# gnosisguild/stylus-zkvm-verifiers

Measured on NVIDIA B200. Metric: groth16_verifies_per_sec, higher is better.
Workload: dtype u256 (8x32-bit Montgomery limbs, IMAD.WIDE.U32)

## Files before the change

stylus_zkvm_verifiers_b200/csrc/kernels.cuh:

```cuda
#pragma once
#include "bn254.cuh"
#include "lazy.cuh"
#include "sha256.cuh"

namespace zkv {

enum : uint8_t { F_INVALID = 1, F_SKIP0 = 2, F_SKIPC = 4, F_SKIPX = 8, F_SELMIS = 16, F_BADDATA = 32 };
enum : uint8_t { ST_OK = 0, ST_INVALID_INITIALIZATION = 1, ST_INVALID_PROOF_DATA = 2, ST_SELECTOR_MISMATCH = 3, ST_VERIFICATION_FAILED = 4 };

__device__ __forceinline__ uint8_t reject_status(uint8_t fl) { return (fl & F_BADDATA) ? ST_INVALID_PROOF_DATA : (fl & F_SELMIS) ? ST_SELECTOR_MISMATCH : ST_VERIFICATION_FAILED; }
#define F_REJECT (F_INVALID | F_SELMIS | F_BADDATA)

#define ZKV_WIN_BITS 4
#define ZKV_WIN_PER_SCALAR 64
#define ZKV_WIN_ENTRIES 15

struct g1aff { fp x, y; };

__device__ __forceinline__ int g1_decode_raw(fp& x, fp& y, const uint32_t* rx, const uint32_t* ry) {
    if (u256_geq(rx, C_P) || u256_geq(ry, C_P)) return 2;
    uint32_t any = 0;
    for (int i = 0; i < 8; i++) any |= rx[i] | ry[i];
    if (!any) { x = fp_zero(); y = fp_zero(); return 1; }
    fp t;
// ... 54 lines not shown
    const uint8_t* rec = rec_off ? recs + (size_t)(rec_off[i] - rec_base) : recs + (size_t)i * stride;
    const uint64_t len = rec_off ? rec_off[i + 1] - rec_off[i] : (uint64_t)stride;
    uint8_t fl = 0;
    if (rec_off && len < 4) fl = F_BADDATA;
    else if (check_selector) {
        uint32_t s = (uint32_t)rec[0] | (uint32_t)rec[1] << 8 | (uint32_t)rec[2] << 16 | (uint32_t)rec[3] << 24;
        if (s != selector_le) fl = F_SELMIS;
    }
    if (rec_off && !fl && len != off + 256) fl = F_BADDATA;
    if (fl) { decode_reject(i, fl, ax, ay, bx, by, cx, cy, flags); return; }
    decode_points(i, rec + off, vm, ax, ay, bx, by, cx, cy, flags);
}

struct Risc0HashConsts { uint32_t tag_out[8], claim_mid[8], sys0[8]; };
__global__ void k_risc0_signals(int n, const uint8_t* image_ids, const uint8_t* journals, const uint8_t* claims, int mode,
                                Risc0HashConsts hc, uint32_t* scal ) {
    int i = blockIdx.x * blockDim.x + threadIdx.x;
    if (i >= n) return;
    uint32_t claim[8];
    if (mode == 0) {
        uint32_t im[8], jr[8];
        for (int k = 0; k < 8; k++) { im[k] = load_be32(image_ids + 32 * (size_t)i + 4 * k); jr[k] = load_be32(journals + 32 * (size_t)i + 4 * k); }
        risc0_claim_digest(claim, im, jr, hc.tag_out, hc.claim_mid, hc.sys0);
    } else {
        for (int k = 0; k < 8; k++) claim[k] = load_be32(claims + 32 * (size_t)i + 4 * k);
    }
    uint32_t* o = scal + (size_t)i * 16;
    for (int k = 0; k < 4; k++) { o[k] = __byte_perm(claim[k], 0, 0x0123); o[8 + k] = __byte_perm(claim[4 + k], 0, 0x0123); o[4 + k] = 0; o[12 + k] = 0; }
}

__global__ void k_sp1_signals(int n, const uint8_t* vkeys, const uint8_t* pv, const uint64_t* pv_off, uint64_t pv_base, size_t pv_stride,
                              uint32_t* scal , uint8_t* flags) {
    int i = blockIdx.x * blockDim.x + threadIdx.x;
    if (i >= n) return;
    uint32_t* o = scal + (size_t)i * 16;
    uint32_t s0[8];
    be32_to_raw(s0, vkeys + 32 * (size_t)i);
    if (u256_geq(s0, C_R)) flags[i] |= F_INVALID;
    for (int k = 0; k < 8; k++) o[k] = s0[k];
    const uint8_t* msg; size_t len;
    if (pv_off) { msg = pv + (size_t)(pv_off[i] - pv_base); len = (size_t)(pv_off[i + 1] - pv_off[i]); } else { msg = pv + (size_t)i * pv_stride; len = pv_stride; }
    uint32_t h[8];
    sha256_msg(h, msg, len);
    h[0] &= 0x1fffffffu;
    for (int k = 0; k < 8; k++) o[8 + k] = h[7 - k];
}

__global__ void k_generic_signals(int n, int k, const uint8_t* sig, uint32_t* scal, uint8_t* flags) {
    int i = blockIdx.x * blockDim.x + threadIdx.x;
    if (i >= n) return;
    bool bad = false;
    for (int j = 0; j < k; j++) {
        uint32_t s[8];
        be32_to_raw(s, sig + ((size_t)i * k + j) * 32);
        bad |= u256_geq(s, C_R);
        for (int t = 0; t < 8; t++) scal[((size_t)i * k + j) * 8 + t] = s[t];
    }
    if (bad) flags[i] |= F_INVALID;
}

__device__ __forceinline__ void vkx_one(int i, const uint32_t* scal, int stride, int ns, int nwin, const g1aff* tab, const g1aff& base, fp* vx, fp* vy, uint8_t* flags) {
    g1j acc;
    if (fp_is_zero(base.x) && fp_is_zero(base.y)) { acc.x = fp_one(); acc.y = fp_one(); acc.z = fp_zero(); }
    else { acc.x = base.x; acc.y = base.y; acc.z = fp_one(); }
    for (int t = 0; t < ns; t++) {
        const uint32_t* s = scal + ((size_t)i * stride + t) * 8;
        const g1aff* tt = tab + (size_t)t * ZKV_WIN_PER_SCALAR * ZKV_WIN_ENTRIES;
        for (int w = 0; w < nwin; w++) {
            uint32_t d = (s[w >> 3] >> ((w & 7) * 4)) & 15u;
            if (d) {
                const g1aff* e = tt + w * ZKV_WIN_ENTRIES + (d - 1);
                fp ex = e->x, ey = e->y;
                if (!(fp_is_zero(ex) && fp_is_zero(ey))) g1_add_affine(acc, ex, ey);
            }
        }
    }
    fp x, y;
    bool fin = g1_to_affine(x, y, acc);
    vx[i] = x; vy[i] = y;
    if (!fin && flags) flags[i] |= F_SKIPX;
}
__global__ void k_vkx(int n, const uint32_t* scal, int ns, int nwin, const g1aff* tab, g1aff base, fp* vx, fp* vy, uint8_t* flags) {
    int i = blockIdx.x * blockDim.x + threadIdx.x;
    if (i >= n) return;
    vkx_one(i, scal, ns, ns, nwin, tab, base, vx, vy, flags);
}

#if defined(__CUDACC__)
__device__ __noinline__ bool g2v_in_subgroup(fp2 qx, fp2 qy) {
    fp2 X = qx, Y = qy, Z = f2_one();
    const fp2 ny = f2v_neg(qy);
    for (int i = ZKV_U_NAF_LEN - 2; i >= 0; i--) {
        {
            fp2 A = f2v_sqr(X), B = f2v_sqr(Y), C = f2v_sqr(B);
            fp2 D = f2v_dbl(f2v_sub(f2v_sub(f2v_sqr(f2v_add(X, B)), A), C));
            fp2 E = f2v_add(f2v_dbl(A), A), F = f2v_sqr(E);
            fp2 X3 = f2v_sub(F, f2v_dbl(D));
            fp2 Y3 = f2v_sub(f2v_mul(E, f2v_sub(D, X3)), f2v_dbl(f2v_dbl(f2v_dbl(C))));
            Z = f2v_dbl(f2v_mul(Y, Z)); X = X3; Y = Y3;
        }
        const int d = C_U_NAF[i];
        if (d) {
            const fp2 ay = d > 0 ? qy : ny;
            if (f2_is_zero(Z)) { X = qx; Y = ay; Z = f2_one(); continue; }
            fp2 z1z1 = f2v_sqr(Z), u2 = f2v_mul(qx, z1z1), s2 = f2v_mul(f2v_mul(ay, Z), z1z1);
            fp2 h = f2v_sub(u2, X), rr = f2v_sub(s2, Y);
            if (f2_is_zero(h)) {
                if (f2_is_zero(rr)) { g2j p, r; p.x = X; p.y = Y; p.z = Z; g2_dbl(r, p); X = r.x; Y = r.y; Z = r.z; }
                else { X = f2_one(); Y = f2_one(); Z = f2_zero(); }
                continue;
            }
            fp2 hh = f2v_sqr(h), hhh = f2v_mul(hh, h), v = f2v_mul(X, hh);
            fp2 X3 = f2v_sub(f2v_sub(f2v_sqr(rr), hhh), f2v_dbl(v));
            fp2 Y3 = f2v_sub(f2v_mul(rr, f2v_sub(v, X3)), f2v_mul(Y, hhh));
            Z = f2v_mul(Z, h); X = X3; Y = Y3;
        }
    }
    g2j q, uq, lhs, t, p1, p2, p3;
    q.x = qx; q.y = qy; q.z = f2_one(); uq.x = X; uq.y = Y; uq.z = Z;
    g2_add(lhs, uq, q);
    g2_psi(p1, uq, 1); g2_add(t, lhs, p1); lhs = t;
    g2_psi(p2, uq, 2); g2_add(t, lhs, p2); lhs = t;
    g2_dbl(t, uq); g2_psi(p3, t, 3);
    return g2j_eq(lhs, p3);
}
#else
static inline bool g2v_in_subgroup(fp2 qx, fp2 qy) { return g2_in_subgroup(qx, qy); }
#endif
__global__ void k_g2_check(int n, const fp2* bx, const fp2* by, uint8_t* flags) {
    int i = blockIdx.x * blockDim.x + threadIdx.x;
    if (i >= n) return;
    uint8_t fl = flags[i];
    if (fl & F_REJECT) return;
    fp2 x = bx[i], y = by[i];
    if (f2_is_zero(x) && f2_is_zero(y)) return;
    if (!g2v_in_subgroup(x, y)) flags[i] = fl | F_INVALID;
}
__global__ void k_g2_target(int n, const fp2* bx, const fp2* by, fp2* tx, fp2* ty) {
    int i = blockIdx.x * blockDim.x + threadIdx.x;
    if (i >= n) return;
    fp2 x = bx[i], y = by[i];
    g2_neg_psi3(x, y);
    tx[i] = x; ty[i] = y;
}

__global__ void k_or_flags(int n, uint8_t* flags, const uint8_t* extra) {
    int i = blockIdx.x * blockDim.x + threadIdx.x;
    if (i < n && extra[i]) flags[i] |= extra[i];
}

struct MillerArgs {
    const fp* px[4]; const fp* py[4];
    const fp2* qx; const fp2* qy;
    const line_t* tabs[3];
    int nfixed;
    const nline_t* ntabs[2];
    const fp12* pre;
    uint8_t skip_bit[4];
    uint8_t vk_skip;
};
#ifndef ZKV_HTPB
#define ZKV_HTPB 128
#endif
#ifndef ZKV_MINBLOCKS
#define ZKV_MINBLOCKS 2
#endif
#define LZ_SMEM_BYTES (LZ_SLOTS * 32 * LZ_NT)
#define LZ_SMEM_MILLER (LZ_SMEM_BYTES + 1024)
__device__ __noinline__ void lz_slopes_to(fp* sl, const fp* x1, const fp* y1, const fp* x2, const fp* y2, bool off1, bool off2) {
    fp x12[2] = {*x1, *x2}, y12[2] = {*y1, *y2}, xy[2], iy[2];
    bool off[2] = {off1, off2};
    g1_slopes2(xy, iy, x12, y12, off);
    sl[0] = xy[0]; sl[1] = xy[1]; sl[2] = iy[0]; sl[3] = iy[1];
}
__device__ __forceinline__ void miller_lz(int n, const MillerArgs& a, const nline_t* nt0, const nline_t* nt1, const fp12* pre, uint8_t vk_skip,
                                          uint8_t* flags, const fp2* tx, const fp2* ty, fp12* fio, g2j* rst, fp* sl, int d_hi, int d_lo, int first, int last) {
    const int i0 = blockIdx.x * LZ_NT + threadIdx.x, i = i0 < n ? i0 : n - 1;
    const uint8_t fl = flags[i];
    uint32_t skip = vk_skip;
    for (int j = 0; j < 3; j++) if (fl & a.skip_bit[j]) skip |= 1u << j;
    if (fl & F_REJECT) skip = 0xF;
    fp* mysl = sl + 4 * (size_t)i0;
    if (first) lz_slopes_to(mysl, a.px[1] + i, a.py[1] + i, a.px[2] + i, a.py[2] + i, (skip & 2u) != 0, (skip & 4u) != 0);
    LzMillerIn in;
    in.px0 = a.px[0] + i; in.py0 = a.py[0] + i; in.qx = a.qx + i; in.qy = a.qy + i; in.sl = mysl; in.nt[0] = nt0; in.nt[1] = nt1; in.var_off = (skip & 1u) != 0;
    const uint32_t tid = lz_tid();
    if (first) lz_miller_init(a.qx[i], a.qy[i]);
    else {
        lz_ldg12(tid + LZ_F * LZ_SLOT, fio + i);
        const g2j* R = rst + i;
        lz_st2(tid + LZ_R * LZ_SLOT, R->x); lz_st2(tid + (LZ_R + 2) * LZ_SLOT, R->y); lz_st2(tid + (LZ_R + 4) * LZ_SLOT, R->z);
    }
    lz_miller_norm_seg(in, d_hi, d_lo, last != 0);
    if (last && !lz_r_is(tid + LZ_R * LZ_SLOT, tx[i], ty[i]) && i0 < n) flags[i] = fl | F_INVALID;
    if (last) { if (pre) lz_f12mul_g(tid + LZ_F * LZ_SLOT, tid + LZ_T * LZ_SLOT, tid + LZ_R * LZ_SLOT, pre, false); }
    else if (i0 < n) { g2j* R = rst + i; R->x = lz_ld2(tid + LZ_R * LZ_SLOT); R->y = lz_ld2(tid + (LZ_R + 2) * LZ_SLOT); R->z = lz_ld2(tid + (LZ_R + 4) * LZ_SLOT); }
    if (i0 < n) lz_stg12(fio + i, tid + LZ_F * LZ_SLOT);
}
__global__ void __launch_bounds__(LZ_NT, 2) k_miller_lz(int n, MillerArgs a, uint8_t* flags, const fp2* tx, const fp2* ty, fp12* fio, g2j* rst, fp* sl, int d_hi, int d_lo, int first, int last) {
    miller_lz(n, a, a.ntabs[0], a.ntabs[1], a.pre, a.vk_skip, flags, tx, ty, fio, rst, sl, d_hi, d_lo, first, last);
}
__device__ __forceinline__ void final_exp_lz(int n, int s_lo, int s_hi, const fp12* in, fp12* st, const uint8_t* flags, uint8_t* status, uint8_t* gt_out, int pairing_mode) {
    const int i0 = blockIdx.x * LZ_NT + threadIdx.x, i = i0 < n ? i0 : n - 1;
    for (int s = s_lo; s <= s_hi; s++) lz_final_exp_stage(s, in + i, st + 6 * (size_t)i0);
    if (s_hi < 3 || i0 >= n) return;
    const uint8_t fl = flags[i];
    if (fl & (pairing_mode ? (F_INVALID | F_SELMIS) : F_REJECT)) {
        status[i] = pairing_mode ? 2 : reject_status(fl);
        if (gt_out) for (int k = 0; k < 384; k++) gt_out[(size_t)i * 384 + k] = 0;
        return;
    }
    const uint32_t tid = lz_tid();
    fp one = fp_one(); uint32_t t = 0;
    for (int k = 0; k < 12; k++) {
        fp w = lz_ldfp(tid + (LZ_A + k) * LZ_SLOT);
        for (int j = 0; j < 8; j++) t |= w.v[j] ^ (k == 0 ? one.v[j] : 0u);
        if (gt_out) fp_to_be32(gt_out + (size_t)i * 384 + 32 * k, w);
    }
    status[i] = pairing_mode ? (t == 0 ? 1 : 0) : (t == 0 ? ST_OK : ST_VERIFICATION_FAILED);
}
__global__ void __launch_bounds__(LZ_NT, 2) k_final_exp_lz(int n, int s_lo, int s_hi, const fp12* in, fp12* st, const uint8_t* flags, uint8_t* status, uint8_t* gt_out, int pairing_mode) {
    final_exp_lz(n, s_lo, s_hi, in, st, flags, status, gt_out, pairing_mode);
}
__global__ void __launch_bounds__(LZ_NT, 2) k_pairing_lz(int n, LzGenIn in, fp12* fio, int d_hi, int d_lo, int first, int last) {
    const size_t i = (size_t)blockIdx.x * LZ_NT + threadIdx.x;
    const uint32_t tid = lz_tid();
    if (first) { fp2 z = f2_zero(); lz_st2(tid + LZ_F * LZ_SLOT, f2_one()); for (int k = 1; k < 6; k++) lz_st2(tid + (LZ_F + 2 * k) * LZ_SLOT, z); }
    else lz_ldg12(tid + LZ_F * LZ_SLOT, fio + i);
    lz_miller_gen_seg(in, i, d_hi, d_lo, first != 0, last != 0);
    lz_stg12(fio + i, tid + LZ_F * LZ_SLOT);
    (void)n;
}
__global__ void k_pairing4_skip(int n, size_t stride, const uint8_t* flags, uint8_t vk_skip, uint8_t* pskip) {
    int i = blockIdx.x * blockDim.x + threadIdx.x;
    if (i >= n) return;
    const uint8_t fl = flags[i], bits[4] = {F_SKIP0, 0x20, 0x40, 0x80};
    const bool bad = (fl & (F_INVALID | F_SELMIS)) != 0;
    for (int j = 0; j < 4; j++) pskip[(size_t)j * stride + i] = (bad || (fl & bits[j]) || ((vk_skip >> j) & 1)) ? 1 : 0;
}
__global__ void k_pairing_decode(int n, int k, size_t stride, const uint8_t* in, fp* px, fp* py, fp2* qx, fp2* qy, uint8_t* pst) {
    size_t t = (size_t)blockIdx.x * blockDim.x + threadIdx.x;
    if (t >= (size_t)n * k) return;
    const size_t i = t / k; const int j = (int)(t % k);
    const uint8_t* p = in + (i * k + j) * 192;
    uint32_t rx[8], ry[8];
    be32_to_raw(rx, p); be32_to_raw(ry, p + 32);
    fp x, y; int r1 = g1_decode_raw(x, y, rx, ry);
    fp2 x2, y2; int r2 = g2_decode_bytes(x2, y2, p + 64);
    const size_t o = (size_t)j * stride + i;
    px[o] = x; py[o] = y; qx[o] = x2; qy[o] = y2;
    pst[o] = (r1 == 2 || r2 == 2) ? F_INVALID : (r1 == 1 || r2 == 1) ? F_SKIP0 : 0;
}
__global__ void k_pairing_flags(int n, int k, size_t stride, const uint8_t* pst, uint8_t* pskip, uint8_t* iflags) {
    int i = blockIdx.x * blockDim.x + threadIdx.x;
    if (i >= n) return;
    uint8_t bad = 0;
    for (int j = 0; j < k; j++) bad |= pst[(size_t)j * stride + i] & F_INVALID;
    for (int j = 0; j < k; j++) pskip[(size_t)j * stride + i] = (bad || (pst[(size_t)j * stride + i] & F_SKIP0)) ? 1 : 0;
    iflags[i] = bad ? F_INVALID : 0;
}
__global__ void __launch_bounds__(ZKV_HTPB, ZKV_MINBLOCKS) k_fp12_op(int n, int op, const uint8_t* a, const uint8_t* b, uint8_t* out) {
    int i0 = blockIdx.x * blockDim.x + threadIdx.x;
    int i = i0 < n ? i0 : n - 1;
    fp12 x, y, z; fp* xw = &x.c0.c0.c0; fp* yw = &y.c0.c0.c0;
    for (int k = 0; k < 12; k++) {
        fp t; be32_to_raw(t.v, a + (size_t)i * 384 + 32 * k); fp_to_mont(xw[k], t);
        if (b) { be32_to_raw(t.v, b + (size_t)i * 384 + 32 * k); fp_to_mont(yw[k], t); } else yw[k] = fp_zero();
    }
    switch (op) {
        case 0: f12_mul(z, x, y); break;
        case 1: f12_sqr(z, x); break;
        case 2: z = x; f12_mul_line(z, y.c0.c0, y.c0.c1, y.c0.c2); break;
        case 3: f12_cyc_sqr(z, x); break;
        case 4: f12_inv(z, x); break;
        case 5: case 6: case 7: f12_frob(z, x, op - 4); break;
        case 8: final_exp(z, x); break;
        default: {
            fp px[1] = {yw[0]}, py[1] = {yw[1]}; fp2 qx, qy; qx.c1 = yw[2]; qx.c0 = yw[3]; qy.c1 = yw[4]; qy.c0 = yw[5];
            miller_loop(z, px, py, qx, qy, nullptr, 0, n > (1 << 30) ? 1u : 0u); break; }
    }
    if (i0 < n) f12_to_bytes(out + (size_t)i * 384, z);
}
__global__ void __launch_bounds__(LZ_NT, 2) k_lz_fp12_op(int n, int op, const uint8_t* a, const uint8_t* b, uint8_t* out, fp12* scratch , const nline_t* ztab) {
    const int i0 = blockIdx.x * LZ_NT + threadIdx.x, i = i0 < n ? i0 : n - 1;
    const uint32_t tid = lz_tid(), A = tid + LZ_A * LZ_SLOT, X = tid + LZ_X * LZ_SLOT, Y = tid + LZ_Y * LZ_SLOT, L = tid + LZ_L * LZ_SLOT;
    fp12* my = scratch + 7 * (size_t)i0;
    {
        fp12 y; fp* yw = &y.c0.c0.c0;
        for (int k = 0; k < 12; k++) {
            fp t; be32_to_raw(t.v, a + (size_t)i * 384 + 32 * k); fp_to_mont(t, t); lz_stfp(A + k * LZ_SLOT, t);
            if (b) { be32_to_raw(t.v, b + (size_t)i * 384 + 32 * k); fp_to_mont(yw[k], t); } else yw[k] = fp_zero();
        }
        my[6] = y;
    }
    switch (op) {
        case 0: lz_f12mul_g(A, X, Y, my + 6, false); break;
        case 1: lz_f12sqr(A, X); break;
        case 2: { fp2 l0 = my[6].c0.c0; lz_st2(L, my[6].c0.c1); lz_st2(L + 2 * LZ_SLOT, my[6].c0.c2); lz_mul_line(A, X, L, l0); break; }
        case 3: lz_cyc_sqr(A, L); break;
        case 4: lz_f12inv(A, X, Y); break;
        case 5: case 6: case 7: lz_frob(A, op - 4); break;
        case 8: { lz_stg12(my + 6, A); for (int s = 0; s < 4; s++) lz_final_exp_stage(s, my + 6, my); break; }
        case 9: lz_st2(L, my[6].c0.c0); lz_st2(L + 2 * LZ_SLOT, my[6].c0.c1); lz_mul_nline(A, X, L); break;
        default: {
            const fp* yw = &my[6].c0.c0.c0;
            fp* g = &my[0].c0.c0.c0;
            g[0] = yw[0]; g[1] = yw[1]; for (int k = 2; k < 6; k++) g[k] = fp_zero();
            fp2 qx, qy; qx.c1 = yw[2]; qx.c0 = yw[3]; qy.c1 = yw[4]; qy.c0 = yw[5];
            fp2* gq = (fp2*)(g + 6); gq[0] = qx; gq[1] = qy;
            LzMillerIn in; in.px0 = g; in.py0 = g + 1; in.sl = g + 2; in.qx = gq; in.qy = gq + 1; in.nt[0] = ztab; in.nt[1] = ztab; in.var_off = false;
            lz_miller_init(qx, qy);
            const int top = ZKV_ATE_NAF_LEN - 2;
            for (int k = 0; k < 3; k++) lz_miller_norm_seg(in, top - (top + 1) * k / 3, top - (top + 1) * (k + 1) / 3 + 1, k == 2);
            break; }
    }
    if (i0 < n) for (int k = 0; k < 12; k++) fp_to_be32(out + (size_t)i * 384 + 32 * k, lz_ldfp(A + k * LZ_SLOT));
}
__global__ void k_f12_to_bytes(int n, const fp12* in, uint8_t* out) {
    int i = blockIdx.x * blockDim.x + threadIdx.x;
    if (i < n) { fp12 t = in[i]; f12_to_bytes(out + (size_t)i * 384, t); }
}

struct VkDev {
    fp2 g2x[3], g2y[3];
    fp alpha_x, alpha_y;
    int valid;
    int g2_inf[3]; int alpha_inf;
    int norm_ok;
};
__global__ void k_vk_setup(const uint8_t* alpha, const uint8_t* g2bytes , VkDev* vk, line_t* lines , nline_t* nlines ) {
    int j = blockIdx.x;
    if (j < 3) {
        fp2 x, y;
        int r = g2_decode_bytes(x, y, g2bytes + 128 * j);
        if (r == 0 && !g2_in_subgroup(x, y)) r = 2;
        vk->g2x[j] = x; vk->g2y[j] = y; vk->g2_inf[j] = (r == 1);
        if (r == 2) atomicAnd(&vk->valid, 0);
        if (r == 0) g2_precompute_lines(lines + (size_t)j * ZKV_LINES_PER_G2, x, y);
        if (j >= 1 && r == 0 && !g2_normalise_lines(nlines + (size_t)(j - 1) * ZKV_LINES_PER_G2, lines + (size_t)j * ZKV_LINES_PER_G2, ZKV_LINES_PER_G2)) atomicAnd(&vk->norm_ok, 0);
    } else if (j == 3) {
        uint32_t rx[8], ry[8]; be32_to_raw(rx, alpha); be32_to_raw(ry, alpha + 32);
        fp x, y; int r = g1_decode_raw(x, y, rx, ry);
        vk->alpha_x = x; vk->alpha_y = y; vk->alpha_inf = (r == 1);
        if (r == 2) atomicAnd(&vk->valid, 0);
    }
}
__global__ void k_vk_miller_ab(const VkDev* vk, const line_t* lines, fp12* out) {
    fp12 f;
    if (vk->alpha_inf || vk->g2_inf[0] || !vk->valid) { f = f12_one(); }
    else {
        fp px[2], py[2]; px[1] = vk->alpha_x; py[1] = vk->alpha_y; px[0] = fp_zero(); py[0] = fp_zero();
        const line_t* tabs[1] = {lines};
        fp2 z = f2_zero();
        miller_loop(f, px, py, z, z, tabs, 1, 1u);
    }
    *out = f;
}
__global__ void k_ic_tables(const uint8_t* ic , g1aff* tab, g1aff* ic0, VkDev* vk) {
    int t = blockIdx.x, w = threadIdx.x;
    uint32_t rx[8], ry[8];
    if (t == 0 && w == 0) {
        be32_to_raw(rx, ic); be32_to_raw(ry, ic + 32);
        fp x, y; int r = g1_decode_raw(x, y, rx, ry);
        if (r == 2) atomicAnd(&vk->valid, 0);
        ic0->x = x; ic0->y = y;
    }
    be32_to_raw(rx, ic + 64 * (t + 1)); be32_to_raw(ry, ic + 64 * (t + 1) + 32);
    fp x, y; int r = g1_decode_raw(x, y, rx, ry);
    if (r == 2 && w == 0) atomicAnd(&vk->valid, 0);
    g1aff* o = tab + ((size_t)t * ZKV_WIN_PER_SCALAR + w) * ZKV_WIN_ENTRIES;
    if (r != 0) { for (int d = 0; d < ZKV_WIN_ENTRIES; d++) { o[d].x = fp_zero(); o[d].y = fp_zero(); } return; }
    g1j b; b.x = x; b.y = y; b.z = fp_one();
    for (int k = 0; k < ZKV_WIN_BITS * w; k++) { g1j d; g1_dbl(d, b); b = d; }
    fp bx, by; g1_to_affine(bx, by, b);
    g1j acc; acc.x = fp_one(); acc.y = fp_one(); acc.z = fp_zero();
    for (int d = 0; d < ZKV_WIN_ENTRIES; d++) {
        g1_add_affine(acc, bx, by);
        fp ex, ey; g1_to_affine(ex, ey, acc);
        o[d].x = ex; o[d].y = ey;
    }
}

#define ZKV_MAX_KEYS 256
#define ZKV_GROUP_TILE 4096
#define ZKV_SLOT_EMPTY 0xffffffffu
struct KeyDesc {
    g1aff base;
    const g1aff* tab;
    const nline_t* nt[2];
    const fp12* pre;
    int ns, vm, reject;
    uint8_t vk_skip;
};
__device__ __forceinline__ uint32_t group_of(uint32_t k, int nk) { return k < (uint32_t)nk ? k : 0u; }
__global__ void __launch_bounds__(256) k_group_count(int n, int nk, const uint32_t* key_idx, uint32_t* cnt) {
    __shared__ uint32_t h[ZKV_MAX_KEYS];
    for (int k = threadIdx.x; k < nk; k += blockDim.x) h[k] = 0;
    __syncthreads();
    const size_t t0 = (size_t)blockIdx.x * ZKV_GROUP_TILE;
    for (int j = threadIdx.x; j < ZKV_GROUP_TILE; j += blockDim.x)
        if (t0 + j < (size_t)n) atomicAdd(&h[group_of(key_idx[t0 + j], nk)], 1u);
    __syncthreads();
    for (int k = threadIdx.x; k < nk; k += blockDim.x) cnt[(size_t)blockIdx.x * nk + k] = h[k];
}
__global__ void __launch_bounds__(ZKV_MAX_KEYS) k_group_scan(int ntiles, int nk, uint32_t* cnt, uint8_t* slot_key, uint32_t* total) {
    __shared__ uint32_t sc[ZKV_MAX_KEYS];
    const int k = threadIdx.x;
    uint32_t c = 0;
    if (k < nk) for (int t = 0; t < ntiles; t++) c += cnt[(size_t)t * nk + k];
    const uint32_t padded = (c + 31u) & ~31u;
    sc[k] = k < nk ? padded : 0u;
    __syncthreads();
    for (int d = 1; d < ZKV_MAX_KEYS; d <<= 1) {
        const uint32_t v = k >= d ? sc[k - d] : 0u;
        __syncthreads();
        sc[k] += v;
        __syncthreads();
    }
    if (k == ZKV_MAX_KEYS - 1) *total = sc[k];
    if (k >= nk) return;
    uint32_t s = sc[k] - padded;
    for (uint32_t p = s + c; p < s + padded; p++) slot_key[p] = (uint8_t)k;
    for (int t = 0; t < ntiles; t++) { const uint32_t v = cnt[(size_t)t * nk + k]; cnt[(size_t)t * nk + k] = s; s += v; }
}
__global__ void __launch_bounds__(256) k_group_scatter(int n, int nk, const uint32_t* key_idx, const uint32_t* base, uint32_t* perm, uint8_t* slot_key) {
    __shared__ uint32_t wc[8][ZKV_MAX_KEYS];
    const int w = threadIdx.x >> 5, lane = threadIdx.x & 31;
    for (int k = lane; k < nk; k += 32) wc[w][k] = 0;
    __syncwarp();
    const size_t r0 = (size_t)blockIdx.x * ZKV_GROUP_TILE + (size_t)w * (ZKV_GROUP_TILE / 8);
    const unsigned lt = (1u << lane) - 1u;
    for (int r = 0; r < ZKV_GROUP_TILE / 8; r += 32) {
        const size_t i = r0 + r + lane;
        const uint32_t k = i < (size_t)n ? group_of(key_idx[i], nk) : ZKV_SLOT_EMPTY;
        const unsigned peers = __match_any_sync(0xffffffffu, k);
        if (k != ZKV_SLOT_EMPTY && (peers & lt) == 0) wc[w][k] += __popc(peers);
        __syncwarp();
    }
    __syncthreads();
    for (int k = threadIdx.x; k < nk; k += blockDim.x) {
        uint32_t run = base[(size_t)blockIdx.x * nk + k];
        for (int v = 0; v < 8; v++) { const uint32_t c = wc[v][k]; wc[v][k] = run; run += c; }
    }
    __syncthreads();
    for (int r = 0; r < ZKV_GROUP_TILE / 8; r += 32) {
        const size_t i = r0 + r + lane;
        const uint32_t k = i < (size_t)n ? group_of(key_idx[i], nk) : ZKV_SLOT_EMPTY;
        const unsigned peers = __match_any_sync(0xffffffffu, k);
        if (k != ZKV_SLOT_EMPTY) { const uint32_t s = wc[w][k] + __popc(peers & lt); perm[s] = (uint32_t)i; slot_key[s] = (uint8_t)k; }
        __syncwarp();
        if (k != ZKV_SLOT_EMPTY && (peers & lt) == 0) wc[w][k] += __popc(peers);
        __syncwarp();
    }
}
__global__ void k_decode_keys(int n, const uint32_t* perm, const uint8_t* slot_key, const KeyDesc* keys, int nk, const uint32_t* key_idx, const uint8_t* proofs,
                              fp* ax, fp* ay, fp2* bx, fp2* by, fp* cx, fp* cy, uint8_t* flags) {
    int i = blockIdx.x * blockDim.x + threadIdx.x;
    if (i >= n) return;
    const uint32_t p = perm[i];
    const KeyDesc* kd = keys + slot_key[i];
    if (p == ZKV_SLOT_EMPTY || key_idx[p] >= (uint32_t)nk || kd->reject) { decode_reject(i, F_INVALID, ax, ay, bx, by, cx, cy, flags); return; }
    decode_points(i, proofs + (size_t)p * 256, kd->vm, ax, ay, bx, by, cx, cy, flags);
}
__global__ void k_signals_keys(int n, const uint32_t* perm, const uint8_t* slot_key, const KeyDesc* keys, const uint8_t* sig, const uint64_t* sig_off, uint64_t sig_base,
                               int stride, uint32_t* scal, uint8_t* flags) {
    int i = blockIdx.x * blockDim.x + threadIdx.x;
    if (i >= n) return;
    const uint32_t p = perm[i];
    if (p == ZKV_SLOT_EMPTY) return;
    const int k = keys[slot_key[i]].ns;
    const uint64_t a = sig_off[p], b = sig_off[p + 1];
    if (b < a || b - a != (uint64_t)k) { flags[i] |= F_INVALID; return; }
    bool bad = false;
    for (int j = 0; j < k; j++) {
        uint32_t s[8];
        be32_to_raw(s, sig + (a - sig_base + j) * 32);
        bad |= u256_geq(s, C_R);
        for (int t = 0; t < 8; t++) scal[((size_t)i * stride + j) * 8 + t] = s[t];
    }
    if (bad) flags[i] |= F_INVALID;
}
__global__ void k_vkx_keys(int n, const uint32_t* perm, const uint8_t* slot_key, const KeyDesc* keys, const uint32_t* scal, int stride, fp* vx, fp* vy, uint8_t* flags) {
    int i = blockIdx.x * blockDim.x + threadIdx.x;
    if (i >= n) return;
    if (perm[i] == ZKV_SLOT_EMPTY) { vx[i] = fp_zero(); vy[i] = fp_zero(); return; }
    const KeyDesc* kd = keys + slot_key[i];
    const g1aff base = kd->base;
    vkx_one(i, scal, stride, kd->ns, ZKV_WIN_PER_SCALAR, kd->tab, base, vx, vy, flags);
}
__device__ __forceinline__ int grouped_in_chunk(const uint32_t* total, size_t o, int m) {
    const size_t t = *total;
    return t <= o ? 0 : (int)(t - o < (size_t)m ? t - o : (size_t)m);
}
__global__ void __launch_bounds__(LZ_NT, 2) k_miller_lz_keys(const uint32_t* total, size_t o, int m, MillerArgs a, const uint8_t* slot_key, const KeyDesc* keys,
                                                            uint8_t* flags, const fp2* tx, const fp2* ty, fp12* fio, g2j* rst, fp* sl, int d_hi, int d_lo, int first, int last) {
    const int n = grouped_in_chunk(total, o, m);
    if ((int)blockIdx.x * LZ_NT >= n) return;
    const int i0 = blockIdx.x * LZ_NT + threadIdx.x;
    const KeyDesc* kd = keys + slot_key[i0 < n ? i0 : n - 1];
    miller_lz(n, a, kd->nt[0], kd->nt[1], kd->pre, kd->vk_skip, flags, tx, ty, fio, rst, sl, d_hi, d_lo, first, last);
}
__global__ void __launch_bounds__(LZ_NT, 2) k_final_exp_lz_keys(const uint32_t* total, size_t o, int m, int s_lo, int s_hi, const fp12* in, fp12* st, const uint8_t* flags, uint8_t* status) {
    const int n = grouped_in_chunk(total, o, m);
    if ((int)blockIdx.x * LZ_NT >= n) return;
    final_exp_lz(n, s_lo, s_hi, in, st, flags, status, nullptr, 0);
}
__global__ void k_status_to_caller(int n, const uint32_t* total, const uint32_t* perm, const uint8_t* slot_status, uint8_t* status) {
    int i = blockIdx.x * blockDim.x + threadIdx.x;
    if (i >= n || (uint32_t)i >= *total) return;
    const uint32_t p = perm[i];
    if (p != ZKV_SLOT_EMPTY) status[p] = slot_status[i];
}

__global__ void k_g1_decode4(int n, const uint8_t* g1s , const uint8_t* g2s ,
                             fp* px0, fp* py0, fp* px1, fp* py1, fp* px2, fp* py2, fp* px3, fp* py3, fp2* qx, fp2* qy, uint8_t* flags) {
    int i = blockIdx.x * blockDim.x + threadIdx.x;
    if (i >= n) return;
    fp* xs[4] = {px0, px1, px2, px3}; fp* ys[4] = {py0, py1, py2, py3};
    const uint8_t bits[4] = {F_SKIP0, 0x20, 0x40, 0x80};
    uint8_t fl = 0;
    for (int j = 0; j < 4; j++) {
        uint32_t rx[8], ry[8];
        const uint8_t* p = g1s + ((size_t)i * 4 + j) * 64;
        be32_to_raw(rx, p); be32_to_raw(ry, p + 32);
        fp x, y; int r = g1_decode_raw(x, y, rx, ry);
        xs[j][i] = x; ys[j][i] = y;
        if (r == 2) fl |= F_INVALID;
        if (r == 1) fl |= bits[j];
    }
    fp2 x2, y2; int rb = g2_decode_bytes(x2, y2, g2s + (size_t)i * 128);
    qx[i] = x2; qy[i] = y2;
    if (rb == 2) fl |= F_INVALID;
    if (rb == 1) fl |= F_SKIP0;
    flags[i] = fl;
}
__global__ void k_fp_mul_bytes(int n, const uint8_t* a, const uint8_t* b, uint8_t* out) {
    int i = blockIdx.x * blockDim.x + threadIdx.x;
    if (i >= n) return;
    fp x, y, z;
    be32_to_raw(x.v, a + 32 * (size_t)i); be32_to_raw(y.v, b + 32 * (size_t)i);
    fp_to_mont(x, x); fp_to_mont(y, y); fp_mul(z, x, y);
    fp_to_be32(out + 32 * (size_t)i, z);
}
__global__ void k_g2_check_bytes(int n, const uint8_t* g2s, uint8_t* out) {
    int i = blockIdx.x * blockDim.x + threadIdx.x;
    if (i >= n) return;
    fp2 x, y; int r = g2_decode_bytes(x, y, g2s + 128 * (size_t)i);
    if (r == 2) { out[i] = 2; return; }
    if (r == 1) { out[i] = 1; return; }
    out[i] = g2_in_subgroup(x, y) ? 1 : 0;
}
__global__ void k_points_to_bytes(int n, const fp* x, const fp* y, uint8_t* out) {
    int i = blockIdx.x * blockDim.x + threadIdx.x;
    if (i >= n) return;
    fp_to_be32(out + 64 * (size_t)i, x[i]); fp_to_be32(out + 64 * (size_t)i + 32, y[i]);
}


__global__ void k_ec_add(int n, const uint8_t* in, uint8_t* out, uint8_t* ok) {
    int i = blockIdx.x * blockDim.x + threadIdx.x;
    if (i >= n) return;
    const uint8_t* p = in + 128 * (size_t)i;
    uint32_t rx[8], ry[8];
    fp x1, y1, x2, y2;
    be32_to_raw(rx, p); be32_to_raw(ry, p + 32);
    int r1 = g1_decode_raw(x1, y1, rx, ry);
    be32_to_raw(rx, p + 64); be32_to_raw(ry, p + 96);
    int r2 = g1_decode_raw(x2, y2, rx, ry);
    uint8_t* o = out + 64 * (size_t)i;
    if (r1 == 2 || r2 == 2) { ok[i] = 1; for (int k = 0; k < 64; k++) o[k] = 0; return; }
    g1j acc;
    if (r1 == 1) { acc.x = fp_one(); acc.y = fp_one(); acc.z = fp_zero(); } else { acc.x = x1; acc.y = y1; acc.z = fp_one(); }
    if (r2 == 0) g1_add_affine(acc, x2, y2);
    fp x, y; g1_to_affine(x, y, acc);
    fp_to_be32(o, x); fp_to_be32(o + 32, y); ok[i] = 0;
}
__global__ void k_ec_mul(int n, const uint8_t* in, uint8_t* out, uint8_t* ok) {
    int i = blockIdx.x * blockDim.x + threadIdx.x;
    if (i >= n) return;
    const uint8_t* p = in + 96 * (size_t)i;
    uint32_t rx[8], ry[8], s[8];
    fp x1, y1;
    be32_to_raw(rx, p); be32_to_raw(ry, p + 32); be32_to_raw(s, p + 64);
    int r1 = g1_decode_raw(x1, y1, rx, ry);
    uint8_t* o = out + 64 * (size_t)i;
    if (r1 == 2) { ok[i] = 1; for (int k = 0; k < 64; k++) o[k] = 0; return; }
    g1j acc; acc.x = fp_one(); acc.y = fp_one(); acc.z = fp_zero();
    if (r1 == 0) {
        for (int b = 255; b >= 0; b--) {
            g1j d; g1_dbl(d, acc); acc = d;
            if ((s[b >> 5] >> (b & 31)) & 1u) g1_add_affine(acc, x1, y1);
        }
    }
    fp x, y; g1_to_affine(x, y, acc);
    fp_to_be32(o, x); fp_to_be32(o + 32, y); ok[i] = 0;
}
__global__ void k_g2_mul(int n, const uint8_t* pts , int bcast, const uint8_t* scalars, uint8_t* out, uint8_t* ok) {
    int i = blockIdx.x * blockDim.x + threadIdx.x;
    if (i >= n) return;
    fp2 qx, qy; uint32_t s[8];
    int r = g2_decode_bytes(qx, qy, pts + (bcast ? 0 : 128 * (size_t)i));
    be32_to_raw(s, scalars + 32 * (size_t)i);
    uint8_t* o = out + 128 * (size_t)i;
    if (r == 2) { ok[i] = 1; for (int k = 0; k < 128; k++) o[k] = 0; return; }
    g2j acc; acc.x = f2_one(); acc.y = f2_one(); acc.z = f2_zero();
    if (r == 0) {
// ... 39 lines not shown
```

stylus_zkvm_verifiers_b200/csrc/lazy.cuh:

```cuda
#pragma once
#include "bn254.cuh"
#if !defined(__CUDACC__)
#include <cstdio>
#include <cstdlib>
#endif

#ifndef LZ_NT
#define LZ_NT 128
#endif
#define LZ_SLOT (2 * LZ_NT)
#define LZ_SLOTS 28

namespace zkv {

#ifdef LZ_LOCKSTEP
#define LZ_RDV() ZKV_RENDEZVOUS()
#else
#define LZ_RDV()
#endif

struct fp4 { fp2 c0, c1; };

#if defined(__CUDACC__)
#ifndef LZ_FN
#define LZ_FN __device__ __noinline__
#endif
#ifndef LZ_FN2
#define LZ_FN2 __device__ __noinline__
#endif
#define LZ_INL __device__ __forceinline__
extern __shared__ uint4 lz_sm[];
LZ_INL uint32_t lz_tid() { return threadIdx.x; }
#ifdef ZKV_LZ_CHECK
#define LZ_CHK(idx) do { if ((idx) + LZ_NT >= LZ_SLOTS * LZ_SLOT) { printf("smem index out of range: %u (thread %u)\n", (unsigned)(idx), threadIdx.x); return; } } while (0)
#else
#define LZ_CHK(idx)
#endif
LZ_INL void lz_ld(uint32_t* r, uint32_t idx) {
    LZ_CHK(idx);
    uint4 a = lz_sm[idx], b = lz_sm[idx + LZ_NT];
    r[0] = a.x; r[1] = a.y; r[2] = a.z; r[3] = a.w; r[4] = b.x; r[5] = b.y; r[6] = b.z; r[7] = b.w;
}
LZ_INL void lz_st(uint32_t idx, const uint32_t* r) {
    LZ_CHK(idx);
    lz_sm[idx] = make_uint4(r[0], r[1], r[2], r[3]); lz_sm[idx + LZ_NT] = make_uint4(r[4], r[5], r[6], r[7]);
}
#else
#include "../../tests/host_emu/lazy_leaf_host.h"
#endif

LZ_INL void lz_fp_neg(uint32_t* r, const uint32_t* a) { fp z = fp_zero(), x, y; for (int i = 0; i < 8; i++) x.v[i] = a[i]; fp_sub(y, z, x); for (int i = 0; i < 8; i++) r[i] = y.v[i]; }

#include "lazy_gen.cuh"

LZ_INL fp lz_ldfp(uint32_t idx) { fp r; lz_ld(r.v, idx); return r; }
LZ_INL void lz_stfp(uint32_t idx, const fp& a) { lz_st(idx, a.v); }
LZ_INL fp2 lz_ld2(uint32_t idx) { fp2 r; lz_ld(r.c0.v, idx); lz_ld(r.c1.v, idx + LZ_SLOT); return r; }
LZ_INL void lz_st2(uint32_t idx, const fp2& a) { lz_st(idx, a.c0.v); lz_st(idx + LZ_SLOT, a.c1.v); }
LZ_INL void lz_st6(uint32_t idx, const fp6& a) { lz_st2(idx, a.c0); lz_st2(idx + 2 * LZ_SLOT, a.c1); lz_st2(idx + 4 * LZ_SLOT, a.c2); }
LZ_INL fp2 f2v_add(const fp2& a, const fp2& b) { fp2 r; f2_add(r, a, b); return r; }
LZ_INL fp2 f2v_sub(const fp2& a, const fp2& b) { fp2 r; f2_sub(r, a, b); return r; }
LZ_INL fp2 f2v_dbl(const fp2& a) { fp2 r; f2_dbl(r, a); return r; }
LZ_INL fp2 f2v_xi(const fp2& a) {
    fp t0, t1; fp2 r;
    fp_dbl(t0, a.c0); fp_dbl(t0, t0); fp_dbl(t0, t0); fp_add(t0, t0, a.c0);
    fp_dbl(t1, a.c1); fp_dbl(t1, t1); fp_dbl(t1, t1); fp_add(t1, t1, a.c1);
    fp_sub(r.c0, t0, a.c1); fp_add(r.c1, t1, a.c0);
    return r;
}

LZ_FN2 void lz_f12sqr(uint32_t f, uint32_t t) {
    LZ_RDV();
    {
        fp6 ab = lz_f6mul(f, f + 6 * LZ_SLOT);
        lz_st6(t, ab);
    }
    {
        fp2 x0 = lz_ld2(f), x1 = lz_ld2(f + 2 * LZ_SLOT), x2 = lz_ld2(f + 4 * LZ_SLOT);
        fp2 y0 = lz_ld2(f + 6 * LZ_SLOT), y1 = lz_ld2(f + 8 * LZ_SLOT), y2 = lz_ld2(f + 10 * LZ_SLOT);
        lz_st2(f, f2v_add(x0, y0)); lz_st2(f + 2 * LZ_SLOT, f2v_add(x1, y1)); lz_st2(f + 4 * LZ_SLOT, f2v_add(x2, y2));
        lz_st2(f + 6 * LZ_SLOT, f2v_add(x0, f2v_xi(y2))); lz_st2(f + 8 * LZ_SLOT, f2v_add(x1, y0)); lz_st2(f + 10 * LZ_SLOT, f2v_add(x2, y1));
    }
    LZ_RDV();
    fp6 p = lz_f6mul(f, f + 6 * LZ_SLOT);
    fp2 t0 = lz_ld2(t), t1 = lz_ld2(t + 2 * LZ_SLOT), t2 = lz_ld2(t + 4 * LZ_SLOT);
    lz_st2(f, f2v_sub(f2v_sub(p.c0, t0), f2v_xi(t2)));
    lz_st2(f + 2 * LZ_SLOT, f2v_sub(f2v_sub(p.c1, t1), t0));
    lz_st2(f + 4 * LZ_SLOT, f2v_sub(f2v_sub(p.c2, t2), t1));
    lz_st2(f + 6 * LZ_SLOT, f2v_dbl(t0)); lz_st2(f + 8 * LZ_SLOT, f2v_dbl(t1)); lz_st2(f + 10 * LZ_SLOT, f2v_dbl(t2));
}

LZ_FN2 void lz_mul_nline(uint32_t f, uint32_t t, uint32_t l) {
    LZ_RDV();
    { fp6 a = lz_f6mul01(f + 6 * LZ_SLOT, l); lz_st6(t, a); }
    fp6 b = lz_f6mul01(f, l);
    lz_st2(f + 6 * LZ_SLOT, f2v_add(lz_ld2(f + 6 * LZ_SLOT), b.c0));
    lz_st2(f + 8 * LZ_SLOT, f2v_add(lz_ld2(f + 8 * LZ_SLOT), b.c1));
    lz_st2(f + 10 * LZ_SLOT, f2v_add(lz_ld2(f + 10 * LZ_SLOT), b.c2));
    lz_st2(f, f2v_add(lz_ld2(f), f2v_xi(lz_ld2(t + 4 * LZ_SLOT))));
    lz_st2(f + 2 * LZ_SLOT, f2v_add(lz_ld2(f + 2 * LZ_SLOT), lz_ld2(t)));
    lz_st2(f + 4 * LZ_SLOT, f2v_add(lz_ld2(f + 4 * LZ_SLOT), lz_ld2(t + 2 * LZ_SLOT)));
}

LZ_FN fp2 f2v_mul(fp2 a, fp2 b) {
    fp2 r;
#if defined(__CUDA_ARCH__)
    fp2_mul_ptx(r.c0.v, r.c1.v, a.c0.v, a.c1.v, b.c0.v, b.c1.v);
#else
    f2_mul(r, a, b);
#endif
    return r;
}
LZ_FN fp2 f2v_sqr(fp2 a) {
    fp2 r;
#if defined(__CUDA_ARCH__)
    fp2_sqr_ptx(r.c0.v, r.c1.v, a.c0.v, a.c1.v);
#else
    f2_sqr(r, a);
#endif
    return r;
}
LZ_INL fp2 f2v_neg(const fp2& a) { fp2 r; f2_neg(r, a); return r; }
LZ_INL fp2 f2v_half(const fp2& a) { fp2 r; f2_half(r, a); return r; }
LZ_INL fp2 f2v_mul_fp(const fp2& a, const fp& k) { fp2 r; fp_mul(r.c0, a.c0, k); fp_mul(r.c1, a.c1, k); return r; }

LZ_FN2 void lz_mul_line(uint32_t f, uint32_t t, uint32_t l, fp2 a) {
    LZ_RDV();
    { fp6 t1 = lz_f6mul01(f + 6 * LZ_SLOT, l); lz_st6(t, t1); }
    for (int k = 0; k < 3; k++) lz_st2(f + (6 + 2 * k) * LZ_SLOT, f2v_add(lz_ld2(f + 2 * k * LZ_SLOT), lz_ld2(f + (6 + 2 * k) * LZ_SLOT)));
    lz_st2(l, f2v_add(lz_ld2(l), a));
    fp6 s = lz_f6mul01(f + 6 * LZ_SLOT, l);
    {
        fp2 t0 = f2v_mul(lz_ld2(f), a), t10 = lz_ld2(t), t12 = lz_ld2(t + 4 * LZ_SLOT);
        lz_st2(f, f2v_add(t0, f2v_xi(t12)));
        lz_st2(f + 6 * LZ_SLOT, f2v_sub(f2v_sub(s.c0, t0), t10));
        t0 = f2v_mul(lz_ld2(f + 2 * LZ_SLOT), a); fp2 t11 = lz_ld2(t + 2 * LZ_SLOT);
        lz_st2(f + 2 * LZ_SLOT, f2v_add(t0, t10));
        lz_st2(f + 8 * LZ_SLOT, f2v_sub(f2v_sub(s.c1, t0), t11));
        t0 = f2v_mul(lz_ld2(f + 4 * LZ_SLOT), a);
        lz_st2(f + 4 * LZ_SLOT, f2v_add(t0, t11));
        lz_st2(f + 10 * LZ_SLOT, f2v_sub(f2v_sub(s.c2, t0), t12));
    }
}

LZ_INL fp2 lz_line_out(uint32_t l, const fp2& l0, const fp2& l3, const fp2& l4, const fp& px, const fp& py, bool off) {
    fp2 a = f2v_mul_fp(l0, py), b = f2v_mul_fp(l3, px), c = l4;
    const uint32_t keep = off ? 0u : 0xffffffffu;
    for (int k = 0; k < 8; k++) {
        a.c0.v[k] = (a.c0.v[k] & keep) | (C_ONE[k] & ~keep); a.c1.v[k] &= keep;
        b.c0.v[k] &= keep; b.c1.v[k] &= keep; c.c0.v[k] &= keep; c.c1.v[k] &= keep;
    }
    lz_st2(l, b); lz_st2(l + 2 * LZ_SLOT, c);
    return a;
}
LZ_FN2 fp2 lz_line_dbl(uint32_t r, uint32_t l, const fp* px, const fp* py, bool off) {
    LZ_RDV();
    fp2 X = lz_ld2(r), Y = lz_ld2(r + 2 * LZ_SLOT), Z = lz_ld2(r + 4 * LZ_SLOT);
    fp2 A = f2v_half(f2v_mul(X, Y));
    fp2 B = f2v_sqr(Y), C = f2v_sqr(Z);
    fp2 E = f2v_mul(f2_const(C_TWIST_B), f2v_add(f2v_dbl(C), C));
    fp2 F = f2v_add(f2v_dbl(E), E);
    fp2 H = f2v_sub(f2v_sqr(f2v_add(Y, Z)), f2v_add(B, C));
    fp2 J = f2v_sqr(X);
    fp2 E2 = f2v_sqr(E);
    lz_st2(r, f2v_mul(A, f2v_sub(B, F)));
    fp2 G = f2v_sqr(f2v_half(f2v_add(B, F)));
    lz_st2(r + 2 * LZ_SLOT, f2v_sub(G, f2v_add(f2v_dbl(E2), E2)));
    lz_st2(r + 4 * LZ_SLOT, f2v_mul(B, H));
    return lz_line_out(l, f2v_neg(H), f2v_add(f2v_dbl(J), J), f2v_sub(E, B), *px, *py, off);
}
LZ_FN2 fp2 lz_line_add(uint32_t r, uint32_t l, fp2 qx, fp2 qy, const fp* px, const fp* py, bool off) {
    LZ_RDV();
    fp2 X = lz_ld2(r), Y = lz_ld2(r + 2 * LZ_SLOT), Z = lz_ld2(r + 4 * LZ_SLOT);
    fp2 th = f2v_sub(Y, f2v_mul(qy, Z)), la = f2v_sub(X, f2v_mul(qx, Z));
    fp2 C = f2v_sqr(th), D = f2v_sqr(la);
    fp2 E = f2v_mul(la, D), F = f2v_mul(Z, C), G = f2v_mul(X, D);
    fp2 H = f2v_sub(f2v_add(E, F), f2v_dbl(G));
    fp2 l4 = f2v_sub(f2v_mul(th, qx), f2v_mul(la, qy));
    lz_st2(r + 2 * LZ_SLOT, f2v_sub(f2v_mul(th, f2v_sub(G, H)), f2v_mul(E, Y)));
    lz_st2(r, f2v_mul(la, H));
    lz_st2(r + 4 * LZ_SLOT, f2v_mul(Z, E));
    return lz_line_out(l, la, f2v_neg(th), l4, *px, *py, off);
}

#define LZ_F 0
#define LZ_T 12
#define LZ_R 18
#define LZ_L 24
struct LzMillerIn {
    const fp *px0, *py0;
    const fp2 *qx, *qy;
    const fp* sl;
    const nline_t* nt[2];
    bool var_off;
};
#define LZ_STAGE (LZ_SLOTS * LZ_SLOT)
#if defined(__CUDACC__)
LZ_INL uint32_t lz_stage_base() { return LZ_STAGE + (lz_tid() >> 5) * 16; }
LZ_INL uint4 lz_line_fetch(const nline_t* const nt[2], int li) {
    const uint32_t lane = lz_tid() & 31;
    uint4 v = make_uint4(0, 0, 0, 0);
    if (lane < 16) v = ((const uint4*)(nt[lane >> 3] + li))[lane & 7];
    return v;
}
LZ_INL void lz_line_stage(uint4 v) {
    const uint32_t lane = lz_tid() & 31;
    __syncwarp();
    if (lane < 16) lz_sm[lz_stage_base() + lane] = v;
    __syncwarp();
}
LZ_INL nline_t lz_line_staged(int j) {
    nline_t nl; uint4* w = (uint4*)&nl;
    for (int k = 0; k < 8; k++) w[k] = lz_sm[lz_stage_base() + 8 * j + k];
    return nl;
}
#else
struct lz_stage_t { nline_t e[2]; };
static lz_stage_t lz_stage_host;
LZ_INL lz_stage_t lz_line_fetch(const nline_t* const nt[2], int li) { lz_stage_t v; v.e[0] = nt[0][li]; v.e[1] = nt[1][li]; return v; }
LZ_INL void lz_line_stage(const lz_stage_t& v) { lz_stage_host = v; }
LZ_INL nline_t lz_line_staged(int j) { return lz_stage_host.e[j]; }
#endif
LZ_INL void lz_fixed_lines(const LzMillerIn& in, int li, uint32_t tid, bool& have) {
    if (!have) lz_line_stage(lz_line_fetch(in.nt, li));
    const int nx = li + 1 < ZKV_LINES_PER_G2 ? li + 1 : li;
    auto next = lz_line_fetch(in.nt, nx);
    for (int j = 0; j < 2; j++) {
        nline_t nl = lz_line_staged(j);
        lz_st2(tid + LZ_L * LZ_SLOT, f2v_mul_fp(nl.n3, in.sl[j]));
        lz_st2(tid + (LZ_L + 2) * LZ_SLOT, f2v_mul_fp(nl.n4, in.sl[2 + j]));
        lz_mul_nline(tid + LZ_F * LZ_SLOT, tid + LZ_T * LZ_SLOT, tid + LZ_L * LZ_SLOT);
    }
    lz_line_stage(next); have = nx == li + 1;
}
LZ_FN2 void lz_miller_norm_seg(LzMillerIn in, int d_hi, int d_lo, bool last) {
    const uint32_t tid = lz_tid(), F = tid + LZ_F * LZ_SLOT, T = tid + LZ_T * LZ_SLOT, RR = tid + LZ_R * LZ_SLOT, L = tid + LZ_L * LZ_SLOT;
    int li = 0; bool have = false;
    for (int d = ZKV_ATE_NAF_LEN - 2; d > d_hi; d--) li += 1 + (C_ATE_NAF[d] != 0);
    for (int d = d_hi; d >= d_lo; d--) {
        if (d != ZKV_ATE_NAF_LEN - 2) lz_f12sqr(F, T);
        { fp2 a = lz_line_dbl(RR, L, in.px0, in.py0, in.var_off); lz_mul_line(F, T, L, a); }
        lz_fixed_lines(in, li, tid, have);
        li++;
        const int dg = C_ATE_NAF[d];
        if (dg) {
            fp2 y = *in.qy; if (dg < 0) y = f2v_neg(y);
            { fp2 a = lz_line_add(RR, L, *in.qx, y, in.px0, in.py0, in.var_off); lz_mul_line(F, T, L, a); }
            lz_fixed_lines(in, li, tid, have);
            li++;
        }
    }
    if (!last) return;
    for (int s = 1; s <= 2; s++) {
        fp2 xs = *in.qx, ys = *in.qy; g2_frob_affine(xs, ys, s);
        if (s == 2) ys = f2v_neg(ys);
        { fp2 a = lz_line_add(RR, L, xs, ys, in.px0, in.py0, in.var_off); lz_mul_line(F, T, L, a); }
        lz_fixed_lines(in, li, tid, have);
        li++;
    }
}
LZ_INL void g2_neg_psi3(fp2& x, fp2& y) {
    f2_conj(x, x); f2_conj(y, y);
    x = f2v_mul(x, f2_const(C_FROB3[2])); y = f2v_neg(f2v_mul(y, f2_const(C_FROB3[3])));
}
LZ_INL bool lz_r_is(uint32_t r, const fp2& tx, const fp2& ty) {
    const fp2 Z = lz_ld2(r + 4 * LZ_SLOT);
    const fp2 dx = f2v_sub(lz_ld2(r), f2v_mul(tx, Z)), dy = f2v_sub(lz_ld2(r + 2 * LZ_SLOT), f2v_mul(ty, Z));
    return (!f2_is_zero(Z) && f2_is_zero(dx) && f2_is_zero(dy)) || (f2_is_zero(tx) && f2_is_zero(ty));
}
struct LzGenIn {
    const fp *px, *py;
    const fp2 *qx, *qy;
    g2j* rst;
    const line_t* tabs[3];
    const uint8_t* pskip;
    size_t stride; int nvar, nfix;
};
LZ_FN2 void lz_miller_gen_seg(LzGenIn in, size_t i, int d_hi, int d_lo, bool first, bool last) {
    const uint32_t tid = lz_tid(), F = tid + LZ_F * LZ_SLOT, T = tid + LZ_T * LZ_SLOT, RR = tid + LZ_R * LZ_SLOT, L = tid + LZ_L * LZ_SLOT;
    const bool keep = in.nvar == 1;
    int li = 0;
    for (int d = ZKV_ATE_NAF_LEN - 2; d > d_hi; d--) li += 1 + (C_ATE_NAF[d] != 0);
    if (keep) {
        if (first) { lz_st2(RR, in.qx[i]); lz_st2(RR + 2 * LZ_SLOT, in.qy[i]); lz_st2(RR + 4 * LZ_SLOT, f2_one()); }
        else { const g2j* R = in.rst + i; lz_st2(RR, R->x); lz_st2(RR + 2 * LZ_SLOT, R->y); lz_st2(RR + 4 * LZ_SLOT, R->z); }
    }
    const int nsteps = (d_hi - d_lo + 1) + (last ? 2 : 0);
    for (int step = 0; step < nsteps; step++) {
        const int d = d_hi - step;
        const int frob = d < d_lo ? d_lo - d : 0;
        if (!frob && d != ZKV_ATE_NAF_LEN - 2) lz_f12sqr(F, T);
        const int dg = frob ? 1 : C_ATE_NAF[d];
        for (int phase = frob ? 1 : 0; phase < 2; phase++) {
            if (phase == 1 && !dg) break;
            for (int j = 0; j < in.nvar; j++) {
                const size_t ij = (size_t)j * in.stride + i;
                const bool off = in.pskip[ij] != 0;
                if (!keep) {
                    if (first && step == 0 && phase == 0) { lz_st2(RR, in.qx[ij]); lz_st2(RR + 2 * LZ_SLOT, in.qy[ij]); lz_st2(RR + 4 * LZ_SLOT, f2_one()); }
                    else { const g2j* R = in.rst + ij; lz_st2(RR, R->x); lz_st2(RR + 2 * LZ_SLOT, R->y); lz_st2(RR + 4 * LZ_SLOT, R->z); }
                }
                fp2 a;
                if (phase == 0) a = lz_line_dbl(RR, L, in.px + ij, in.py + ij, off);
                else {
                    fp2 x = in.qx[ij], y = in.qy[ij];
                    if (frob) { if (frob == 1) { f2_conj(x, x); f2_conj(y, y); } x = f2v_mul(x, f2_const(frob == 1 ? C_FROB1[2] : C_FROB2[2])); y = f2v_mul(y, f2_const(frob == 1 ? C_FROB1[3] : C_FROB2[3])); if (frob == 2) y = f2v_neg(y); }
                    else if (dg < 0) y = f2v_neg(y);
                    a = lz_line_add(RR, L, x, y, in.px + ij, in.py + ij, off);
                }
                lz_mul_line(F, T, L, a);
                if (!keep) { g2j* R = in.rst + ij; R->x = lz_ld2(RR); R->y = lz_ld2(RR + 2 * LZ_SLOT); R->z = lz_ld2(RR + 4 * LZ_SLOT); }
            }
            for (int j = 0; j < in.nfix; j++) {
                const size_t ij = (size_t)(in.nvar + j) * in.stride + i;
                const line_t ln = in.tabs[j][li];
                fp2 a = lz_line_out(L, ln.l0, ln.l3, ln.l4, in.px[ij], in.py[ij], in.pskip[ij] != 0);
                lz_mul_line(F, T, L, a);
            }
            li++;
        }
    }
    if (keep && !last) { g2j* R = in.rst + i; R->x = lz_ld2(RR); R->y = lz_ld2(RR + 2 * LZ_SLOT); R->z = lz_ld2(RR + 4 * LZ_SLOT); }
}
LZ_INL void lz_miller_init(const fp2& qx, const fp2& qy) {
    const uint32_t tid = lz_tid();
    fp2 one = f2_one(), z = f2_zero();
    lz_st2(tid + LZ_F * LZ_SLOT, one);
    for (int k = 1; k < 6; k++) lz_st2(tid + (LZ_F + 2 * k) * LZ_SLOT, z);
    lz_st2(tid + LZ_R * LZ_SLOT, qx); lz_st2(tid + (LZ_R + 2) * LZ_SLOT, qy); lz_st2(tid + (LZ_R + 4) * LZ_SLOT, one);
}

LZ_INL void lz_ldg6(uint32_t dst, const fp6* src, bool neg) {
    const fp* w = &src->c0.c0;
    for (int k = 0; k < 6; k++) { fp t = w[k]; if (neg) fp_neg(t, t); lz_stfp(dst + k * LZ_SLOT, t); }
}
LZ_INL void lz_ldg12(uint32_t dst, const fp12* src) { lz_ldg6(dst, &src->c0, false); lz_ldg6(dst + 6 * LZ_SLOT, &src->c1, false); }
LZ_INL void lz_stg12(fp12* dst, uint32_t src) { fp* w = &dst->c0.c0.c0; for (int k = 0; k < 12; k++) w[k] = lz_ldfp(src + k * LZ_SLOT); }
LZ_INL void lz_conj(uint32_t a) { for (int k = 6; k < 12; k++) { fp t = lz_ldfp(a + k * LZ_SLOT); fp_neg(t, t); lz_stfp(a + k * LZ_SLOT, t); } }
LZ_FN2 void lz_f12mul_g(uint32_t a, uint32_t x, uint32_t y, const fp12* b, bool conjb) {
    LZ_RDV();
    lz_ldg6(x, &b->c0, false);
    { fp6 t0 = lz_f6mul(a, x); lz_st6(y, t0); }
    for (int k = 0; k < 3; k++) lz_st2(a + 2 * k * LZ_SLOT, f2v_add(lz_ld2(a + 2 * k * LZ_SLOT), lz_ld2(a + (6 + 2 * k) * LZ_SLOT)));
    lz_ldg6(x, &b->c1, conjb);
    { fp6 t1 = lz_f6mul(a + 6 * LZ_SLOT, x); lz_st6(a + 6 * LZ_SLOT, t1); }
    { const fp* w = &b->c0.c0.c0; for (int k = 0; k < 6; k++) { fp t; fp_add(t, lz_ldfp(x + k * LZ_SLOT), w[k]); lz_stfp(x + k * LZ_SLOT, t); } }
    LZ_RDV();
    fp6 m = lz_f6mul(a, x);
    fp2 t10 = lz_ld2(a + 6 * LZ_SLOT), t11 = lz_ld2(a + 8 * LZ_SLOT), t12 = lz_ld2(a + 10 * LZ_SLOT);
    fp2 t00 = lz_ld2(y), t01 = lz_ld2(y + 2 * LZ_SLOT), t02 = lz_ld2(y + 4 * LZ_SLOT);
    lz_st2(a + 6 * LZ_SLOT, f2v_sub(f2v_sub(m.c0, t00), t10));
    lz_st2(a + 8 * LZ_SLOT, f2v_sub(f2v_sub(m.c1, t01), t11));
    lz_st2(a + 10 * LZ_SLOT, f2v_sub(f2v_sub(m.c2, t02), t12));
    lz_st2(a, f2v_add(t00, f2v_xi(t12)));
    lz_st2(a + 2 * LZ_SLOT, f2v_add(t01, t10));
    lz_st2(a + 4 * LZ_SLOT, f2v_add(t02, t11));
}
LZ_FN2 void lz_cyc_sqr(uint32_t a, uint32_t l) {
    LZ_RDV();
    const uint32_t z0 = a, z4 = a + 2 * LZ_SLOT, z3 = a + 4 * LZ_SLOT, z2 = a + 6 * LZ_SLOT, z1 = a + 8 * LZ_SLOT, z5 = a + 10 * LZ_SLOT;
    {
        fp4 t = lz_f4sqr(z0, z1);
        fp2 x = f2v_dbl(f2v_sub(t.c0, lz_ld2(z0))); lz_st2(z0, f2v_add(x, t.c0));
        x = f2v_dbl(f2v_add(t.c1, lz_ld2(z1))); lz_st2(z1, f2v_add(x, t.c1));
    }
    { fp4 t = lz_f4sqr(z2, z3); lz_st2(l, t.c0); lz_st2(l + 2 * LZ_SLOT, t.c1); }
    {
        fp4 t = lz_f4sqr(z4, z5);
        fp2 t5 = f2v_xi(t.c1);
        fp2 x = f2v_dbl(f2v_add(t5, lz_ld2(z2))); lz_st2(z2, f2v_add(x, t5));
        x = f2v_dbl(f2v_sub(t.c0, lz_ld2(z3))); lz_st2(z3, f2v_add(x, t.c0));
        fp2 t2 = lz_ld2(l), t3 = lz_ld2(l + 2 * LZ_SLOT);
        x = f2v_dbl(f2v_sub(t2, lz_ld2(z4))); lz_st2(z4, f2v_add(x, t2));
        x = f2v_dbl(f2v_add(t3, lz_ld2(z5))); lz_st2(z5, f2v_add(x, t3));
    }
}
LZ_FN2 void lz_frob(uint32_t a, int k) {
    LZ_RDV();
    const int slot_of_w[6] = {0, 3, 1, 4, 2, 5};
    for (int i = 0; i < 6; i++) {
        const uint32_t s = a + 2 * slot_of_w[i] * LZ_SLOT;
        fp2 c = lz_ld2(s);
        if (k & 1) f2_conj(c, c);
        if (i) c = f2v_mul(c, (k == 1) ? f2_const(C_FROB1[i]) : (k == 2) ? f2_const(C_FROB2[i]) : f2_const(C_FROB3[i]));
        if (i || (k & 1)) lz_st2(s, c);
    }
}
LZ_INL fp fpv_inv(fp a) { fp r; fp_inv(r, a); return r; }
LZ_FN2 void lz_f12inv(uint32_t a, uint32_t x, uint32_t y) {
    LZ_RDV();
    { fp6 s0 = lz_f6mul(a, a); lz_st6(y, s0); }
    {
        fp6 s1 = lz_f6mul(a + 6 * LZ_SLOT, a + 6 * LZ_SLOT);
        lz_st2(x, f2v_sub(lz_ld2(y), f2v_xi(s1.c2)));
        lz_st2(x + 2 * LZ_SLOT, f2v_sub(lz_ld2(y + 2 * LZ_SLOT), s1.c0));
        lz_st2(x + 4 * LZ_SLOT, f2v_sub(lz_ld2(y + 4 * LZ_SLOT), s1.c1));
    }
    {
        fp2 c0 = lz_ld2(x), c1 = lz_ld2(x + 2 * LZ_SLOT), c2 = lz_ld2(x + 4 * LZ_SLOT);
        fp2 A = f2v_sub(f2v_sqr(c0), f2v_xi(f2v_mul(c1, c2)));
        fp2 B = f2v_sub(f2v_xi(f2v_sqr(c2)), f2v_mul(c0, c1));
        fp2 C = f2v_sub(f2v_sqr(c1), f2v_mul(c0, c2));
        fp2 F = f2v_add(f2v_add(f2v_mul(c0, A), f2v_xi(f2v_mul(c2, B))), f2v_xi(f2v_mul(c1, C)));
        fp n, t; fp_sqr(n, F.c0); fp_sqr(t, F.c1); fp_add(n, n, t); n = fpv_inv(n);
        fp2 Fi; fp_mul(Fi.c0, F.c0, n); fp_mul(t, F.c1, n); fp_neg(Fi.c1, t);
        lz_st2(x, f2v_mul(A, Fi)); lz_st2(x + 2 * LZ_SLOT, f2v_mul(B, Fi)); lz_st2(x + 4 * LZ_SLOT, f2v_mul(C, Fi));
    }
    LZ_RDV();
    { fp6 r0 = lz_f6mul(a, x); lz_st6(a, r0); }
    {
        fp6 r1 = lz_f6mul(a + 6 * LZ_SLOT, x);
        lz_st2(a + 6 * LZ_SLOT, f2v_neg(r1.c0)); lz_st2(a + 8 * LZ_SLOT, f2v_neg(r1.c1)); lz_st2(a + 10 * LZ_SLOT, f2v_neg(r1.c2));
    }
}
#define LZ_A 0
#define LZ_X 12
#define LZ_Y 18
LZ_INL void lz_pow_u(const fp12* ga, fp12* ga3) {
    const uint32_t tid = lz_tid(), A = tid + LZ_A * LZ_SLOT, X = tid + LZ_X * LZ_SLOT, Y = tid + LZ_Y * LZ_SLOT, L = tid + LZ_L * LZ_SLOT;
    lz_ldg12(A, ga);
    lz_cyc_sqr(A, L); lz_f12mul_g(A, X, Y, ga, false);
    lz_stg12(ga3, A);
    if (C_U_WNAF3[ZKV_U_WNAF3_LEN - 1] == 1) lz_ldg12(A, ga);
    for (int i = ZKV_U_WNAF3_LEN - 2; i >= 0; i--) {
        lz_cyc_sqr(A, L);
        const int d = C_U_WNAF3[i];
        if (d) lz_f12mul_g(A, X, Y, (d == 1 || d == -1) ? ga : ga3, d < 0);
    }
}
LZ_INL void lz_final_exp_stage(int stage, const fp12* m, fp12* st) {
    const uint32_t tid = lz_tid(), A = tid + LZ_A * LZ_SLOT, X = tid + LZ_X * LZ_SLOT, Y = tid + LZ_Y * LZ_SLOT, L = tid + LZ_L * LZ_SLOT;
    fp12 *f = st, *s1 = st + 1, *x = st + 2, *y = st + 3, *z = st + 4, *t = st + 5;
    if (stage == 0) {
        lz_ldg12(A, m); lz_f12inv(A, X, Y); lz_f12mul_g(A, X, Y, m, true);
        lz_stg12(f, A); lz_frob(A, 2); lz_f12mul_g(A, X, Y, f, false);
        lz_stg12(f, A);
        lz_pow_u(f, s1);
        lz_stg12(t, A);
    } else if (stage == 1) {
        lz_ldg12(A, t);
        lz_cyc_sqr(A, L); lz_stg12(x, A);
        lz_cyc_sqr(A, L); lz_f12mul_g(A, X, Y, x, false); lz_stg12(y, A);
        lz_pow_u(y, s1); lz_stg12(z, A);
    } else if (stage == 2) {
        lz_ldg12(A, z);
        lz_cyc_sqr(A, L); lz_stg12(t, A);
        lz_pow_u(t, s1);
        lz_stg12(t, A);
    } else {
        lz_ldg12(A, t);
        lz_f12mul_g(A, X, Y, z, false); lz_f12mul_g(A, X, Y, y, false); lz_stg12(t, A);
        lz_f12mul_g(A, X, Y, x, true); lz_stg12(s1, A);
        lz_frob(A, 1); lz_stg12(x, A);
        lz_ldg12(A, s1); lz_f12mul_g(A, X, Y, f, true); lz_frob(A, 3); lz_stg12(s1, A);
        lz_ldg12(A, t); lz_frob(A, 2); lz_stg12(y, A);
        lz_ldg12(A, t); lz_f12mul_g(A, X, Y, z, false); lz_f12mul_g(A, X, Y, f, false);
        lz_f12mul_g(A, X, Y, x, false); lz_f12mul_g(A, X, Y, y, false); lz_f12mul_g(A, X, Y, s1, false);
    }
}

}
```

stylus_zkvm_verifiers_b200/csrc/zkv.cu:

```cuda
#include <cuda_runtime.h>
#include <algorithm>
#include <cstdio>
#include <cstdlib>
#include <cstring>
#include <atomic>
#include <mutex>
#include <string>
#include <thread>
#include <utility>
#include <vector>

#include "../../include/zkv.h"
#include "kernels.cuh"
#include "vk_constants.h"

using namespace zkv;

static thread_local std::string g_err;
static int fail(int code, const std::string& msg) { g_err = msg; return code; }
#define CK(call)                                                                                       \
    do {                                                                                               \
        cudaError_t e_ = (call);                                                                       \
        if (e_ != cudaSuccess) return fail(ZKV_ERR_CUDA, std::string(#call) + ": " + cudaGetErrorString(e_)); \
    } while (0)
// ... 698 lines not shown
        std::lock_guard<std::mutex> lk(c->mu);
        CK(cudaSetDevice(c->device));
        int rc = ctx_wait_idle(c); if (rc) return rc;
        rc = ctx_reserve(c, 1, 24); if (rc) return rc;
        uint32_t sc[24]; memset(sc, 0, sizeof sc);
        uint8_t w32[32];
        memset(w32, 0, 32); memcpy(w32 + 16, h->control_root_0, 16); for (int k = 0; k < 8; k++) sc[k] = load_be32(w32 + 4 * (7 - k));
        memset(w32, 0, 32); memcpy(w32 + 16, h->control_root_1, 16); for (int k = 0; k < 8; k++) sc[8 + k] = load_be32(w32 + 4 * (7 - k));
        for (int k = 0; k < 8; k++) sc[16 + k] = load_be32(bn254_control_id + 4 * (7 - k));
        CK(cudaMemcpyAsync(c->scal, sc, sizeof sc, cudaMemcpyHostToDevice, c->stream));
        CK(cudaMemsetAsync(c->flags, 0, 1, c->stream));
        if (!h->all_fail && h->vk->valid) {
            k_vkx<<<1, 1, 0, c->stream>>>(1, c->scal, 2, ZKV_WIN_PER_SCALAR, c->d_tab, c->h_ic0, c->px[2], c->py[2], c->flags);
            g1aff mid;
            CK(cudaMemcpyAsync(&mid.x, c->px[2], sizeof(fp), cudaMemcpyDeviceToHost, c->stream)); CK(cudaMemcpyAsync(&mid.y, c->py[2], sizeof(fp), cudaMemcpyDeviceToHost, c->stream));
            CK(cudaStreamSynchronize(c->stream));
            k_vkx<<<1, 1, 0, c->stream>>>(1, c->scal + 16, 1, ZKV_WIN_PER_SCALAR, c->d_tab + (size_t)4 * ZKV_WIN_PER_SCALAR * ZKV_WIN_ENTRIES, mid, c->px[2], c->py[2], c->flags);
            CK(cudaMemcpyAsync(&h->base.x, c->px[2], sizeof(fp), cudaMemcpyDeviceToHost, c->stream)); CK(cudaMemcpyAsync(&h->base.y, c->py[2], sizeof(fp), cudaMemcpyDeviceToHost, c->stream));
            CK(cudaStreamSynchronize(c->stream));
            CK(cudaGetLastError());
        } else memset(&h->base, 0, sizeof h->base);
    }
    h->initialized = 1;
    return 0;
}
extern "C" int zkv_risc0_is_initialized(const zkv_risc0* h) { return h ? h->initialized : 0; }
extern "C" int zkv_risc0_get_selector(const zkv_risc0* h, uint8_t out[4]) { if (!h || !out) return fail(ZKV_ERR_ARG, "null"); if (h->initialized) memcpy(out, h->selector, 4); else memset(out, 0, 4); return 0; }
extern "C" int zkv_risc0_get_control_root(const zkv_risc0* h, uint8_t out0[16], uint8_t out1[16]) {
    if (!h || !out0 || !out1) return fail(ZKV_ERR_ARG, "null");
    if (h->initialized) { memcpy(out0, h->control_root_0, 16); memcpy(out1, h->control_root_1, 16); } else { memset(out0, 0, 16); memset(out1, 0, 16); }
    return 0;
}
extern "C" int zkv_risc0_get_bn254_control_id(const zkv_risc0* h, uint8_t out[32]) { if (!h || !out) return fail(ZKV_ERR_ARG, "null"); if (h->initialized) memcpy(out, h->bn254_control_id, 32); else memset(out, 0, 32); return 0; }
extern "C" int zkv_risc0_get_verifier_key_digest(const zkv_risc0* h, uint8_t out[32]) { if (!h || !out) return fail(ZKV_ERR_ARG, "null"); risc0_vk_digest(out, h->vk); return 0; }

static uint32_t sel_le(const uint8_t s[4]) { return (uint32_t)s[0] | (uint32_t)s[1] << 8 | (uint32_t)s[2] << 16 | (uint32_t)s[3] << 24; }
static int risc0_batch(const zkv_risc0* h, const uint8_t* seals, const uint64_t* seal_off, const uint8_t* a32, const uint8_t* b32, int integrity, size_t n, uint8_t* status_out) {
    if (!h || (n && (!seals || !seal_off || !a32 || (!integrity && !b32) || !status_out))) return fail(ZKV_ERR_ARG, "zkv_risc0_verify_batch: null argument");
    if (n == 0) return 0;
    if (n > 0xffffffffull) return fail(ZKV_ERR_ARG, "batch too large");
    if (!offsets_ok(seal_off, n)) return fail(ZKV_ERR_ARG, "seal offsets must be non-decreasing");
    if (!h->initialized) { memset(status_out, ZKV_INVALID_INITIALIZATION, n); return 0; }
    const zkv_vk* vk = h->vk;
    const bool direct = n >= 4096 && is_pinned(seals) && is_pinned(seal_off) && is_pinned(a32) && (integrity || is_pinned(b32));
    const size_t per = integrity ? 32 : 64;
    return for_each_device(vk->devs, n, [&](DevCtx* c, size_t b, size_t e) -> int {
        return host_pipeline(c, vk, b, e, 2, status_out,
            [&](size_t i0, size_t cnt, Sink* dst) -> size_t {
                const size_t bytes = (size_t)(seal_off[i0 + cnt] - seal_off[i0]);
                if (!dst) return (cnt + 1) * 8 + cnt * per + bytes + 320;
                size_t p = 0;
                dst->put(p, seal_off + i0, (cnt + 1) * 8); p += (cnt + 1) * 8;
                dst->put(p, a32 + i0 * 32, cnt * 32); p += cnt * 32;
                if (!integrity) { dst->put(p, b32 + i0 * 32, cnt * 32); p += cnt * 32; }
                dst->put(p, seals + seal_off[i0], bytes, true); p += bytes;
                return p + 320;
            },
            [&](size_t i0, size_t cnt, uint8_t* d) -> Job {
                Job j;
                j.rec_off = (const uint64_t*)d; j.rec_base = seal_off[i0]; j.off = 4; j.stride = 260; j.check_selector = 1; j.selector_le = sel_le(h->selector);
                j.mode = integrity ? SIG_RISC0_INTEGRITY : SIG_RISC0_VERIFY;
                j.sig_a = d + (cnt + 1) * 8; j.sig_b = j.sig_a + cnt * 32; j.recs = j.sig_a + cnt * per;
                j.hc = h->hc; j.base = h->base; j.all_fail = h->all_fail;
                return j;
            }, direct);
    });
}
extern "C" int zkv_risc0_verify_batch(const zkv_risc0* h, const uint8_t* seals, const uint64_t* seal_off, const uint8_t* image_ids, const uint8_t* journal_digests, size_t n, uint8_t* status_out) {
    return risc0_batch(h, seals, seal_off, image_ids, journal_digests, 0, n, status_out);
}
extern "C" int zkv_risc0_verify_integrity_batch(const zkv_risc0* h, const uint8_t* seals, const uint64_t* seal_off, const uint8_t* claim_digests, size_t n, uint8_t* status_out) {
    return risc0_batch(h, seals, seal_off, claim_digests, nullptr, 1, n, status_out);
}
extern "C" int zkv_risc0_verify(const zkv_risc0* h, const uint8_t* seal, size_t seal_len, const uint8_t image_id[32], const uint8_t journal_digest[32], uint8_t* status_out) {
    uint64_t off[2] = {0, seal_len}; uint8_t dummy = 0;
    return risc0_batch(h, seal ? seal : &dummy, off, image_id, journal_digest, 0, 1, status_out);
}
extern "C" int zkv_risc0_verify_integrity(const zkv_risc0* h, const uint8_t* seal, size_t seal_len, const uint8_t claim_digest[32], uint8_t* status_out) {
    uint64_t off[2] = {0, seal_len}; uint8_t dummy = 0;
    return risc0_batch(h, seal ? seal : &dummy, off, claim_digest, nullptr, 1, 1, status_out);
}
extern "C" int zkv_risc0_verify_batch_device(const zkv_risc0* h, int device, const void* d_seals260, const void* d_image_ids, const void* d_journal_digests, size_t n, void* d_status_out, void* stream) {
    if (!h || !d_seals260 || !d_image_ids || !d_journal_digests || !d_status_out) return fail(ZKV_ERR_ARG, "zkv_risc0_verify_batch_device: null argument");
    DevCtx* c = vk_ctx(h->vk, device);
    if (!c) return fail(ZKV_ERR_ARG, "device not in the handle's device list");
    if (n > MAX_CHUNK * 8) return fail(ZKV_ERR_ARG, "device batch too large");
    if (!h->initialized) {
        CK(cudaSetDevice(device));
        CK(cudaMemsetAsync(d_status_out, ZKV_INVALID_INITIALIZATION, n, (cudaStream_t)stream));
        return 0;
    }
    Job j;
    j.vk = h->vk; j.n = n; j.recs = (const uint8_t*)d_seals260; j.stride = 260; j.off = 4; j.check_selector = 1; j.selector_le = sel_le(h->selector);
    j.mode = SIG_RISC0_VERIFY; j.sig_a = (const uint8_t*)d_image_ids; j.sig_b = (const uint8_t*)d_journal_digests; j.hc = h->hc; j.base = h->base; j.all_fail = h->all_fail;
    j.d_status = (uint8_t*)d_status_out;
    return device_call(c, device, stream, [&](cudaStream_t s) { return run_verify(c, j, s); });
}

struct zkv_sp1 { const zkv_vk* vk = nullptr; zkv_vk* owned = nullptr; uint8_t verifier_hash[32]; };
extern "C" int zkv_sp1_create(const zkv_vk* vk_or_null, const int* devices, int n_dev, zkv_sp1** out) {
    if (!out) return fail(ZKV_ERR_ARG, "zkv_sp1_create: null out");
    zkv_sp1* h = new zkv_sp1();
    memcpy(h->verifier_hash, ZKV_SP1_VERIFIER_HASH, 32);
    if (vk_or_null) { if (vk_or_null->n_ic != 3 || vk_or_null->vm != ZKV_VM_SP1) { delete h; return fail(ZKV_ERR_ARG, "zkv_sp1_create: need a ZKV_VM_SP1 key with 3 IC points"); } h->vk = vk_or_null; }
    else { int rc = zkv_vk_load_sp1(devices, n_dev, &h->owned); if (rc) { delete h; return rc; } h->vk = h->owned; }
    *out = h; return 0;
}
extern "C" void zkv_sp1_destroy(zkv_sp1* h) { if (!h) return; if (h->owned) zkv_vk_free(h->owned); delete h; }
extern "C" int zkv_sp1_verifier_hash(const zkv_sp1* h, uint8_t out[32]) { if (!h || !out) return fail(ZKV_ERR_ARG, "null"); memcpy(out, h->verifier_hash, 32); return 0; }
extern "C" const char* zkv_sp1_version(const zkv_sp1*) { return ZKV_SP1_VERSION; }

extern "C" int zkv_sp1_verify_batch(const zkv_sp1* h, const uint8_t* vkeys, const uint8_t* public_values, const uint64_t* pv_off, const uint8_t* proofs, const uint64_t* proof_off, size_t n, uint8_t* status_out) {
    if (!h || (n && (!vkeys || !public_values || !pv_off || !proofs || !proof_off || !status_out))) return fail(ZKV_ERR_ARG, "zkv_sp1_verify_batch: null argument");
    if (n == 0) return 0;
    if (n > 0xffffffffull) return fail(ZKV_ERR_ARG, "batch too large");
    if (!offsets_ok(proof_off, n) || !offsets_ok(pv_off, n)) return fail(ZKV_ERR_ARG, "proof / public-value offsets must be non-decreasing");
    const zkv_vk* vk = h->vk;
    const bool direct = n >= 4096 && is_pinned(proofs) && is_pinned(proof_off) && is_pinned(pv_off) && is_pinned(vkeys) && is_pinned(public_values);
    return for_each_device(vk->devs, n, [&](DevCtx* c, size_t b, size_t e) -> int {
        return host_pipeline(c, vk, b, e, 2, status_out,
            [&](size_t i0, size_t cnt, Sink* dst) -> size_t {
                const size_t pr = (size_t)(proof_off[i0 + cnt] - proof_off[i0]), pv = (size_t)(pv_off[i0 + cnt] - pv_off[i0]);
                if (!dst) return (cnt + 1) * 16 + cnt * 32 + pr + pv + 320;
                size_t p = 0;
                dst->put(p, proof_off + i0, (cnt + 1) * 8); p += (cnt + 1) * 8;
                dst->put(p, pv_off + i0, (cnt + 1) * 8); p += (cnt + 1) * 8;
                dst->put(p, vkeys + i0 * 32, cnt * 32); p += cnt * 32;
                dst->put(p, proofs + proof_off[i0], pr, true); p += pr;
                dst->put(p, public_values + pv_off[i0], pv, true); p += pv;
                return p + 320;
            },
            [&](size_t i0, size_t cnt, uint8_t* d) -> Job {
                Job j;
                j.rec_off = (const uint64_t*)d; j.rec_base = proof_off[i0]; j.off = 4; j.stride = 260; j.check_selector = 1; j.selector_le = sel_le(h->verifier_hash);
                j.mode = SIG_SP1; j.pv_off = (const uint64_t*)(d + (cnt + 1) * 8); j.pv_base = pv_off[i0];
                j.sig_a = d + (cnt + 1) * 16; j.recs = j.sig_a + cnt * 32; j.sig_b = j.recs + (size_t)(proof_off[i0 + cnt] - proof_off[i0]);
                j.base = c->h_ic0;
                return j;
            }, direct);
    });
}
extern "C" int zkv_sp1_verify_proof(const zkv_sp1* h, const uint8_t vkey[32], const uint8_t* public_values, size_t pv_len, const uint8_t* proof, size_t proof_len, uint8_t* status_out) {
    uint64_t po[2] = {0, proof_len}, vo[2] = {0, pv_len}; uint8_t dummy = 0;
    return zkv_sp1_verify_batch(h, vkey, public_values ? public_values : &dummy, vo, proof ? proof : &dummy, po, 1, status_out);
}
extern "C" int zkv_sp1_verify_batch_device(const zkv_sp1* h, int device, const void* d_vkeys, const void* d_public_values, size_t pv_stride, const void* d_proofs260, size_t n, void* d_status_out, void* stream) {
    if (!h || !d_vkeys || !d_public_values || !d_proofs260 || !d_status_out) return fail(ZKV_ERR_ARG, "zkv_sp1_verify_batch_device: null argument");
    DevCtx* c = vk_ctx(h->vk, device);
    if (!c) return fail(ZKV_ERR_ARG, "device not in the handle's device list");
    if (n > MAX_CHUNK * 8) return fail(ZKV_ERR_ARG, "device batch too large");
    Job j;
    j.vk = h->vk; j.n = n; j.recs = (const uint8_t*)d_proofs260; j.stride = 260; j.off = 4; j.check_selector = 1; j.selector_le = sel_le(h->verifier_hash);
    j.mode = SIG_SP1; j.sig_a = (const uint8_t*)d_vkeys; j.sig_b = (const uint8_t*)d_public_values; j.pv_off = nullptr; j.pv_stride = pv_stride; j.base = c->h_ic0;
    j.d_status = (uint8_t*)d_status_out;
    return device_call(c, device, stream, [&](cudaStream_t s) { return run_verify(c, j, s); });
}


extern "C" void zkv_test_parallel_copy(void* dst, const void* src, size_t n) { pcopy(dst, src, n); }
extern "C" void* zkv_host_alloc(size_t bytes) {
    void* p = nullptr;
    if (zkv_device_count() <= 0 || cudaHostAlloc(&p, bytes ? bytes : 1, cudaHostAllocPortable) != cudaSuccess) { cudaGetLastError(); fail(ZKV_ERR_CUDA, "zkv_host_alloc: cudaHostAlloc failed"); return nullptr; }
    return p;
}
extern "C" void zkv_host_free(void* p) { if (p) cudaFreeHost(p); }

extern "C" int zkv_self_test(int device) {
    if (zkv_device_count() <= device || device < 0) return fail(ZKV_ERR_CUDA, "no such CUDA device (this library has no CPU path)");
    zkv_risc0* r0 = nullptr; zkv_sp1* s1 = nullptr;
    int rc = zkv_risc0_create(nullptr, &device, 1, &r0);
    if (!rc) rc = zkv_risc0_initialize(r0, ZKV_RISC0_FIXTURE_CONTROL_ROOT, ZKV_RISC0_FIXTURE_BN254_CONTROL_ID);
    if (!rc) rc = zkv_sp1_create(nullptr, &device, 1, &s1);
    if (!rc) {
        uint8_t st[4] = {255, 255, 255, 255};
        uint8_t seal[sizeof ZKV_RISC0_FIXTURE_SEAL], proof[sizeof ZKV_SP1_FIXTURE_PROOF];
        memcpy(seal, ZKV_RISC0_FIXTURE_SEAL, sizeof seal); memcpy(proof, ZKV_SP1_FIXTURE_PROOF, sizeof proof);
        rc = zkv_risc0_verify(r0, seal, sizeof seal, ZKV_RISC0_FIXTURE_IMAGE_ID, ZKV_RISC0_FIXTURE_JOURNAL_DIGEST, &st[0]);
        seal[4 + 100] ^= 0x04;
        if (!rc) rc = zkv_risc0_verify(r0, seal, sizeof seal, ZKV_RISC0_FIXTURE_IMAGE_ID, ZKV_RISC0_FIXTURE_JOURNAL_DIGEST, &st[1]);
        if (!rc) rc = zkv_sp1_verify_proof(s1, ZKV_SP1_FIXTURE_VKEY, ZKV_SP1_FIXTURE_PUBLIC_VALUES, sizeof ZKV_SP1_FIXTURE_PUBLIC_VALUES, proof, sizeof proof, &st[2]);
        uint8_t vkey[32]; memcpy(vkey, ZKV_SP1_FIXTURE_VKEY, 32); vkey[31] ^= 1;
        if (!rc) rc = zkv_sp1_verify_proof(s1, vkey, ZKV_SP1_FIXTURE_PUBLIC_VALUES, sizeof ZKV_SP1_FIXTURE_PUBLIC_VALUES, proof, sizeof proof, &st[3]);
        if (!rc && !(st[0] == ZKV_OK && st[2] == ZKV_OK && st[1] != ZKV_OK && st[1] != 255 && st[3] == ZKV_VERIFICATION_FAILED)) {
            char msg[160]; snprintf(msg, sizeof msg, "zkv_self_test: kernels returned statuses %d %d %d %d for the reference's golden proofs and their tampers; expected 0, reject, 0, 1", st[0], st[1], st[2], st[3]);
            rc = fail(ZKV_ERR_STATE, msg);
        }
    }
    if (r0) zkv_risc0_destroy(r0);
    if (s1) zkv_sp1_destroy(s1);
    return rc;
}
static int pairing4_chain(DevCtx* c, size_t o, int n, const uint8_t* d_g1s, const uint8_t* d_g2s, uint8_t* d_ok, uint8_t* d_gt, uint8_t* d_miller, cudaStream_t s, bool timed) {
    uint8_t* flags = c->flags + o;
    if (timed) CK(cudaEventRecord(c->ev[0], s));
    k_g1_decode4<<<nblk(n), TPB, 0, s>>>(n, d_g1s + o * 256, d_g2s + o * 128, c->px[0] + o, c->py[0] + o, c->px[1] + o, c->py[1] + o, c->px[2] + o, c->py[2] + o, c->px[3] + o, c->py[3] + o, c->qx + o, c->qy + o, flags);
    if (timed) { CK(cudaEventRecord(c->ev[1], s)); CK(cudaEventRecord(c->ev[2], s)); }
    k_g2_check<<<nblk(n), TPB, 0, s>>>(n, c->qx + o, c->qy + o, flags);
    if (timed) CK(cudaEventRecord(c->ev[3], s));
    const uint8_t vk_skip = (uint8_t)((c->h_vk.g2_inf[0] ? 2 : 0) | (c->h_vk.g2_inf[1] ? 4 : 0) | (c->h_vk.g2_inf[2] ? 8 : 0));
    k_pairing4_skip<<<nblk(n), TPB, 0, s>>>(n, c->stride, flags, vk_skip, c->pskip + o);
    LzGenIn gi; memset(&gi, 0, sizeof gi);
    gi.px = c->px[0] + o; gi.py = c->py[0] + o; gi.qx = c->qx + o; gi.qy = c->qy + o; gi.rst = c->rst + o; gi.pskip = c->pskip + o; gi.stride = c->stride; gi.nvar = 1; gi.nfix = 3;
    for (int j = 0; j < 3; j++) gi.tabs[j] = c->d_lines + (size_t)j * ZKV_LINES_PER_G2;
    k_pairing_lz<<<nblk(n, LZ_NT), LZ_NT, LZ_SMEM_BYTES, s>>>(n, gi, c->f + o, ZKV_ATE_NAF_LEN - 2, 0, 1, 1);
    if (timed) CK(cudaEventRecord(c->ev[4], s));
    if (d_miller) k_f12_to_bytes<<<nblk(n), TPB, 0, s>>>(n, c->f + o, d_miller + o * 384);
    k_final_exp_lz<<<nblk(n, LZ_NT), LZ_NT, LZ_SMEM_BYTES, s>>>(n, 0, 3, c->f + o, c->fes + 6 * o, flags, d_ok + o, d_gt ? d_gt + o * 384 : nullptr, 1);
    if (timed) CK(cudaEventRecord(c->ev[5], s));
    CK(cudaGetLastError());
    return 0;
}
static int run_pairing4(DevCtx* c, const zkv_vk* vk, size_t n_, const uint8_t* d_g1s, const uint8_t* d_g2s, uint8_t* d_ok, uint8_t* d_gt, uint8_t* d_miller, cudaStream_t s) {
    if (n_ == 0) return 0;
    int rc = ctx_acquire(c, s); if (rc) return rc;
    rc = ctx_reserve(c, n_, 8); if (rc) return rc;
    if (!vk->valid) {
        CK(cudaMemsetAsync(d_ok, 2, n_, s)); if (d_gt) CK(cudaMemsetAsync(d_gt, 0, n_ * 384, s)); if (d_miller) CK(cudaMemsetAsync(d_miller, 0, n_ * 384, s));
        for (int e = 0; e < 6; e++) CK(cudaEventRecord(c->ev[e], s));
        return 0;
    }
    int chunks = chunk_count(c, n_, vk->tune.overlap_chunks.load());
    if (vk->tune.overlap_chunks.load() == 0 && n_ >= 2 * wave_proofs_of(c)) chunks = 1;
    if (chunks <= 1) return pairing4_chain(c, 0, (int)n_, d_g1s, d_g2s, d_ok, d_gt, d_miller, s, true);
    return fork_join(c, s, n_, chunks, [&](size_t o, int m, cudaStream_t st) { return pairing4_chain(c, o, m, d_g1s, d_g2s, d_ok, d_gt, d_miller, st, false); });
}
extern "C" int zkv_pairing4_batch(const zkv_vk* vk, const uint8_t* g1s, const uint8_t* g2s, size_t n, uint8_t* ok_out, uint8_t* gt_out, uint8_t* miller_out) {
    if (!vk || (n && (!g1s || !g2s || !ok_out))) return fail(ZKV_ERR_ARG, "zkv_pairing4_batch: null argument");
    if (n == 0) return 0;
    const size_t CH = (size_t)1 << 18;
    return for_each_device(vk->devs, n, [&](DevCtx* c, size_t b, size_t e) -> int {
        if (int rc = ctx_wait_idle(c)) return rc;
        for (size_t s0 = b; s0 < e; s0 += CH) {
            size_t m = std::min(CH, e - s0);
            size_t ob = m + (gt_out ? m * 384 : 0) + (miller_out ? m * 384 : 0);
            int rc = ctx_stage(c, m * 384, ob); if (rc) return rc;
            memcpy(c->h_pin, g1s + s0 * 256, m * 256); memcpy(c->h_pin + m * 256, g2s + s0 * 128, m * 128);
            CK(cudaMemcpyAsync(c->d_in, c->h_pin, m * 384, cudaMemcpyHostToDevice, c->stream));
            uint8_t* d_gt = gt_out ? c->d_out + m : nullptr; uint8_t* d_ml = miller_out ? c->d_out + m + (gt_out ? m * 384 : 0) : nullptr;
            rc = run_pairing4(c, vk, m, c->d_in, c->d_in + m * 256, c->d_out, d_gt, d_ml, c->stream); if (rc) return rc;
            CK(cudaMemcpyAsync(c->h_out, c->d_out, ob, cudaMemcpyDeviceToHost, c->stream));
            CK(cudaStreamSynchronize(c->stream));
            collect_stage_ms(c);
            memcpy(ok_out + s0, c->h_out, m);
            if (gt_out) memcpy(gt_out + s0 * 384, c->h_out + m, m * 384);
            if (miller_out) memcpy(miller_out + s0 * 384, c->h_out + m + (gt_out ? m * 384 : 0), m * 384);
        }
        return 0;
    });
}
extern "C" int zkv_pairing4_batch_device(const zkv_vk* vk, int device, const void* d_g1s, const void* d_g2s, size_t n, void* d_ok_out, void* d_gt_out, void* stream) {
    if (!vk || !d_g1s || !d_g2s || !d_ok_out) return fail(ZKV_ERR_ARG, "zkv_pairing4_batch_device: null argument");
    DevCtx* c = vk_ctx(vk, device);
    if (!c) return fail(ZKV_ERR_ARG, "device not in the key's device list");
    if (n > MAX_CHUNK * 8) return fail(ZKV_ERR_ARG, "device batch too large");
    return device_call(c, device, stream, [&](cudaStream_t s) {
        return run_pairing4(c, vk, n, (const uint8_t*)d_g1s, (const uint8_t*)d_g2s, (uint8_t*)d_ok_out, (uint8_t*)d_gt_out, nullptr, s);
    });
}

extern "C" int zkv_vk_x_batch(const zkv_vk* vk, const uint8_t* signals, int k, size_t n, uint8_t* out_points) {
    if (!vk || !signals || !out_points || k + 1 != vk->n_ic) return fail(ZKV_ERR_ARG, "zkv_vk_x_batch: bad argument");
    if (n == 0) return 0;
    if (n > MAX_CHUNK * 8) return fail(ZKV_ERR_ARG, "zkv_vk_x_batch: batch too large");
    DevCtx* c = vk->devs[0];
    std::lock_guard<std::mutex> lk(c->mu);
    CK(cudaSetDevice(c->device));
    int rc = ctx_wait_idle(c); if (rc) return rc;
    rc = ctx_reserve(c, n, (size_t)k * 8); if (rc) return rc;
    rc = ctx_stage(c, n * (size_t)k * 32, n * 64); if (rc) return rc;
    CK(cudaMemcpyAsync(c->d_in, signals, n * (size_t)k * 32, cudaMemcpyHostToDevice, c->stream));
    CK(cudaMemsetAsync(c->flags, 0, n, c->stream));
    k_generic_signals<<<nblk(n), TPB, 0, c->stream>>>((int)n, k, c->d_in, c->scal, c->flags);
    k_vkx<<<nblk(n), TPB, 0, c->stream>>>((int)n, c->scal, k, ZKV_WIN_PER_SCALAR, c->d_tab, c->h_ic0, c->px[2], c->py[2], c->flags);
    k_points_to_bytes<<<nblk(n), TPB, 0, c->stream>>>((int)n, c->px[2], c->py[2], c->d_out);
    CK(cudaGetLastError());
    CK(cudaMemcpyAsync(out_points, c->d_out, n * 64, cudaMemcpyDeviceToHost, c->stream));
    CK(cudaStreamSynchronize(c->stream));
    return 0;
}

template <class L>
static int with_scratch(int device, const void* in0, size_t b0, const void* in1, size_t b1, void* out0, size_t ob0, void* out1, size_t ob1, L launch) {
    if (zkv_device_count() <= device || device < 0) return fail(ZKV_ERR_CUDA, "no such CUDA device (this library has no CPU path)");
    CK(cudaSetDevice(device));
    uint8_t *d0 = nullptr, *d1 = nullptr, *o0 = nullptr, *o1 = nullptr;
    CK(cudaMalloc(&d0, b0 + 16)); CK(cudaMalloc(&d1, b1 + 16)); CK(cudaMalloc(&o0, ob0 + 16)); CK(cudaMalloc(&o1, ob1 + 16));
    CK(cudaMemcpy(d0, in0, b0, cudaMemcpyHostToDevice)); if (b1) CK(cudaMemcpy(d1, in1, b1, cudaMemcpyHostToDevice));
    launch(d0, d1, o0, o1);
    cudaError_t e = cudaGetLastError(); if (e == cudaSuccess) e = cudaDeviceSynchronize();
    if (e == cudaSuccess) { e = cudaMemcpy(out0, o0, ob0, cudaMemcpyDeviceToHost); if (e == cudaSuccess && ob1) e = cudaMemcpy(out1, o1, ob1, cudaMemcpyDeviceToHost); }
    cudaFree(d0); cudaFree(d1); cudaFree(o0); cudaFree(o1);
    if (e != cudaSuccess) return fail(ZKV_ERR_CUDA, cudaGetErrorString(e));
    return 0;
}
extern "C" int zkv_fp_mul_batch(const uint8_t* a, const uint8_t* b, size_t n, uint8_t* out, int device) {
    if (!a || !b || !out) return fail(ZKV_ERR_ARG, "null");
    if (n == 0) return 0;
    uint8_t dummy;
    return with_scratch(device, a, n * 32, b, n * 32, out, n * 32, &dummy, 0, [&](uint8_t* d0, uint8_t* d1, uint8_t* o0, uint8_t*) { k_fp_mul_bytes<<<nblk(n), TPB>>>((int)n, d0, d1, o0); });
}
extern "C" int zkv_fp12_op_batch(int op, const uint8_t* a, const uint8_t* b, size_t n, uint8_t* out, int device) {
    const bool slots = op >= 16;
    const int k = slots ? op - 16 : op;
    if (!a || !out || k < 0 || k > (slots ? 10 : 9) || ((k == 0 || k == 2 || k == 9 || k == 10) && !b)) return fail(ZKV_ERR_ARG, "zkv_fp12_op_batch: bad argument");
    if (n == 0) return 0;
    uint8_t dummy;
    if (!slots)
        return with_scratch(device, a, n * 384, b ? b : &dummy, b ? n * 384 : 0, out, n * 384, &dummy, 0,
                            [&](uint8_t* d0, uint8_t* d1, uint8_t* o0, uint8_t*) { k_fp12_op<<<nblk(n, ZKV_HTPB), ZKV_HTPB>>>((int)n, k, d0, b ? d1 : nullptr, o0); });
    const size_t launched = (size_t)nblk(n, LZ_NT) * LZ_NT;
    std::vector<uint8_t> sink(1);
    if (zkv_device_count() <= device || device < 0) return fail(ZKV_ERR_CUDA, "no such CUDA device (this library has no CPU path)");
    CK(cudaSetDevice(device));
    CK(cudaFuncSetAttribute(k_lz_fp12_op, cudaFuncAttributeMaxDynamicSharedMemorySize, LZ_SMEM_MILLER));
    fp12* scratch = nullptr; CK(cudaMalloc(&scratch, launched * 7 * sizeof(fp12)));
    nline_t* ztab = nullptr; CK(cudaMalloc(&ztab, ZKV_LINES_PER_G2 * sizeof(nline_t))); CK(cudaMemset(ztab, 0, ZKV_LINES_PER_G2 * sizeof(nline_t)));
    int rc = with_scratch(device, a, n * 384, b ? b : &dummy, b ? n * 384 : 0, out, n * 384, &dummy, 0,
                          [&](uint8_t* d0, uint8_t* d1, uint8_t* o0, uint8_t*) { k_lz_fp12_op<<<nblk(n, LZ_NT), LZ_NT, LZ_SMEM_MILLER>>>((int)n, k, d0, b ? d1 : nullptr, o0, scratch, ztab); });
    cudaFree(scratch); cudaFree(ztab);
    return rc;
}
extern "C" int zkv_g2_check_batch(const uint8_t* g2s, size_t n, uint8_t* out, int device) {
    if (!g2s || !out) return fail(ZKV_ERR_ARG, "null");
    if (n == 0) return 0;
    uint8_t dummy;
    return with_scratch(device, g2s, n * 128, &dummy, 0, out, n, &dummy, 0, [&](uint8_t* d0, uint8_t*, uint8_t* o0, uint8_t*) { k_g2_check_bytes<<<nblk(n), TPB>>>((int)n, d0, o0); });
}
extern "C" int zkv_ec_add_batch(const uint8_t* in, size_t n, uint8_t* out, uint8_t* reverted, int device) {
    if (!in || !out || !reverted) return fail(ZKV_ERR_ARG, "null");
    if (n == 0) return 0;
    uint8_t dummy;
    return with_scratch(device, in, n * 128, &dummy, 0, out, n * 64, reverted, n, [&](uint8_t* d0, uint8_t*, uint8_t* o0, uint8_t* o1) { k_ec_add<<<nblk(n), TPB>>>((int)n, d0, o0, o1); });
}
extern "C" int zkv_ec_mul_batch(const uint8_t* in, size_t n, uint8_t* out, uint8_t* reverted, int device) {
    if (!in || !out || !reverted) return fail(ZKV_ERR_ARG, "null");
    if (n == 0) return 0;
    uint8_t dummy;
    return with_scratch(device, in, n * 96, &dummy, 0, out, n * 64, reverted, n, [&](uint8_t* d0, uint8_t*, uint8_t* o0, uint8_t* o1) { k_ec_mul<<<nblk(n), TPB>>>((int)n, d0, o0, o1); });
}
extern "C" int zkv_g2_mul_batch(const uint8_t* points, int broadcast_point, const uint8_t* scalars, size_t n, uint8_t* out, uint8_t* reverted, int device) {
    if (!points || !scalars || !out || !reverted) return fail(ZKV_ERR_ARG, "null");
    if (n == 0) return 0;
    return with_scratch(device, points, broadcast_point ? 128 : n * 128, scalars, n * 32, out, n * 128, reverted, n,
                        [&](uint8_t* d0, uint8_t* d1, uint8_t* o0, uint8_t* o1) { k_g2_mul<<<nblk(n), TPB>>>((int)n, d0, broadcast_point, d1, o0, o1); });
}
static int ec_pairing_on(int device, const uint8_t* in, int k, size_t n, uint8_t* out, uint8_t* reverted, uint8_t* miller_out) {
    CK(cudaSetDevice(device));
    CK(cudaFuncSetAttribute(k_pairing_lz, cudaFuncAttributeMaxDynamicSharedMemorySize, LZ_SMEM_BYTES));
    CK(cudaFuncSetAttribute(k_final_exp_lz, cudaFuncAttributeMaxDynamicSharedMemorySize, LZ_SMEM_BYTES));
    const size_t CH = (size_t)1 << 16;
    const size_t cap = std::min(CH, (n + LZ_NT - 1) / LZ_NT * LZ_NT), K = (size_t)k;
    uint8_t *d_in = nullptr, *d_pst = nullptr, *d_pskip = nullptr, *d_ifl = nullptr, *d_st = nullptr, *d_ml = nullptr;
    fp *d_px = nullptr, *d_py = nullptr; fp2 *d_qx = nullptr, *d_qy = nullptr; g2j* d_r = nullptr; fp12 *d_f = nullptr, *d_fes = nullptr;
    auto release = [&]() { cudaFree(d_in); cudaFree(d_pst); cudaFree(d_pskip); cudaFree(d_ifl); cudaFree(d_st); cudaFree(d_ml); cudaFree(d_px); cudaFree(d_py); cudaFree(d_qx); cudaFree(d_qy); cudaFree(d_r); cudaFree(d_f); cudaFree(d_fes); };
#define CKR(call) do { cudaError_t e_ = (call); if (e_ != cudaSuccess) { release(); return fail(ZKV_ERR_CUDA, std::string(#call) + ": " + cudaGetErrorString(e_)); } } while (0)
    CKR(cudaMalloc(&d_in, cap * K * 192)); CKR(cudaMalloc(&d_pst, cap * K)); CKR(cudaMalloc(&d_pskip, cap * K)); CKR(cudaMalloc(&d_ifl, cap)); CKR(cudaMalloc(&d_st, cap));
    CKR(cudaMalloc(&d_px, cap * K * sizeof(fp))); CKR(cudaMalloc(&d_py, cap * K * sizeof(fp))); CKR(cudaMalloc(&d_qx, cap * K * sizeof(fp2))); CKR(cudaMalloc(&d_qy, cap * K * sizeof(fp2)));
    CKR(cudaMalloc(&d_r, cap * K * sizeof(g2j))); CKR(cudaMalloc(&d_f, cap * sizeof(fp12))); CKR(cudaMalloc(&d_fes, cap * 6 * sizeof(fp12)));
    if (miller_out) CKR(cudaMalloc(&d_ml, cap * 384));
    std::vector<uint8_t> h_st(cap), h_ifl(cap);
    for (size_t s0 = 0; s0 < n; s0 += CH) {
        const size_t m = std::min(CH, n - s0);
        const int blocks = nblk(m, LZ_NT);
        CKR(cudaMemcpy(d_in, in + s0 * K * 192, m * K * 192, cudaMemcpyHostToDevice));
        CKR(cudaMemset(d_px, 0, cap * K * sizeof(fp))); CKR(cudaMemset(d_py, 0, cap * K * sizeof(fp))); CKR(cudaMemset(d_qx, 0, cap * K * sizeof(fp2))); CKR(cudaMemset(d_qy, 0, cap * K * sizeof(fp2)));
        CKR(cudaMemset(d_pst, F_SKIP0, cap * K)); CKR(cudaMemset(d_pskip, 1, cap * K));
        k_pairing_decode<<<nblk(m * K), TPB>>>((int)m, k, cap, d_in, d_px, d_py, d_qx, d_qy, d_pst);
        k_g2_check<<<nblk(cap * K), TPB>>>((int)(cap * K), d_qx, d_qy, d_pst);
        k_pairing_flags<<<nblk(m), TPB>>>((int)m, k, cap, d_pst, d_pskip, d_ifl);
        LzGenIn gi; memset(&gi, 0, sizeof gi);
        gi.px = d_px; gi.py = d_py; gi.qx = d_qx; gi.qy = d_qy; gi.rst = d_r; gi.pskip = d_pskip; gi.stride = cap; gi.nvar = k; gi.nfix = 0;
        k_pairing_lz<<<blocks, LZ_NT, LZ_SMEM_BYTES>>>((int)m, gi, d_f, ZKV_ATE_NAF_LEN - 2, 0, 1, 1);
        if (miller_out) k_f12_to_bytes<<<nblk(m), TPB>>>((int)m, d_f, d_ml);
        k_final_exp_lz<<<blocks, LZ_NT, LZ_SMEM_BYTES>>>((int)m, 0, 3, d_f, d_fes, d_ifl, d_st, nullptr, 1);
        CKR(cudaGetLastError());
        CKR(cudaMemcpy(h_st.data(), d_st, m, cudaMemcpyDeviceToHost)); CKR(cudaMemcpy(h_ifl.data(), d_ifl, m, cudaMemcpyDeviceToHost));
        if (miller_out) CKR(cudaMemcpy(miller_out + s0 * 384, d_ml, m * 384, cudaMemcpyDeviceToHost));
        for (size_t t = 0; t < m; t++) {
            uint8_t* o = out + (s0 + t) * 32; memset(o, 0, 32);
            if (h_ifl[t]) { reverted[s0 + t] = 1; if (miller_out) memset(miller_out + (s0 + t) * 384, 0, 384); }
            else { reverted[s0 + t] = 0; o[31] = h_st[t] == 1 ? 1 : 0; }
        }
    }
#undef CKR
    release();
    return 0;
}
extern "C" int zkv_ec_pairing_batch(const uint8_t* in, int k, size_t n, uint8_t* out, uint8_t* reverted, uint8_t* miller_out, int device) {
    if (!out || !reverted || k < 0 || k > 64 || (k && n && !in)) return fail(ZKV_ERR_ARG, "zkv_ec_pairing_batch: bad argument");
    if (n == 0) return 0;
    if (zkv_device_count() <= device || device < 0) return fail(ZKV_ERR_CUDA, "no such CUDA device (this library has no CPU path)");
    if (k == 0) {
        for (size_t i = 0; i < n; i++) { memset(out + 32 * i, 0, 32); out[32 * i + 31] = 1; reverted[i] = 0; }
        if (miller_out) for (size_t i = 0; i < n; i++) { memset(miller_out + 384 * i, 0, 384); miller_out[384 * i + 31] = 1; }
        return 0;
    }
    return ec_pairing_on(device, in, k, n, out, reverted, miller_out);
}
extern "C" int zkv_ec_pairing(const uint8_t* in, size_t len, uint8_t out[32], uint8_t* reverted, int device) {
    if (!out || !reverted || (len && !in)) return fail(ZKV_ERR_ARG, "zkv_ec_pairing: null argument");
    if (len % 192) { memset(out, 0, 32); *reverted = 1; return 0; }
    return zkv_ec_pairing_batch(in, (int)(len / 192), 1, out, reverted, nullptr, device);
}

extern "C" int zkv_last_stage_ms(const void* handle_vk, int device, float* out, int cap) {
    const zkv_vk* vk = (const zkv_vk*)handle_vk;
    if (!vk || !out) return fail(ZKV_ERR_ARG, "null");
    DevCtx* c = vk_ctx(vk, device);
    if (!c) return fail(ZKV_ERR_ARG, "device not in the key's device list");
    std::lock_guard<std::mutex> lk(c->mu);
    if (cudaSetDevice(device) == cudaSuccess) { cudaEventSynchronize(c->ev[5]); collect_stage_ms(c); }
    int m = std::min(cap, 5);
    for (int i = 0; i < m; i++) out[i] = c->stage_ms[i];
    return m;
}
extern "C" const void* zkv_risc0_vk(const zkv_risc0* h) { return h ? h->vk : nullptr; }
extern "C" const void* zkv_sp1_vk(const zkv_sp1* h) { return h ? h->vk : nullptr; }

extern "C" long long zkv_wave_proofs(int device, int kernel) {
    if (zkv_device_count() <= device || device < 0) return fail(ZKV_ERR_CUDA, "no such CUDA device");
    if (cudaSetDevice(device) != cudaSuccess) return fail(ZKV_ERR_CUDA, "cudaSetDevice failed");
    cudaDeviceProp prop; if (cudaGetDeviceProperties(&prop, device) != cudaSuccess) return fail(ZKV_ERR_CUDA, "cudaGetDeviceProperties failed");
    int per_sm = 0;
    cudaError_t e; int tpb;
    switch (kernel) {
        case 0: tpb = LZ_NT; cudaFuncSetAttribute(k_miller_lz, cudaFuncAttributeMaxDynamicSharedMemorySize, LZ_SMEM_MILLER); e = cudaOccupancyMaxActiveBlocksPerMultiprocessor(&per_sm, k_miller_lz, LZ_NT, LZ_SMEM_MILLER); break;
        case 1: tpb = LZ_NT; cudaFuncSetAttribute(k_final_exp_lz, cudaFuncAttributeMaxDynamicSharedMemorySize, LZ_SMEM_BYTES); e = cudaOccupancyMaxActiveBlocksPerMultiprocessor(&per_sm, k_final_exp_lz, LZ_NT, LZ_SMEM_BYTES); break;
        default: return fail(ZKV_ERR_ARG, "zkv_wave_proofs: kernel must be 0 or 1 (2 and 3, the round-1 kernels, were removed)");
    }
    if (e != cudaSuccess) return fail(ZKV_ERR_CUDA, cudaGetErrorString(e));
    return (long long)prop.multiProcessorCount * per_sm * tpb;
}
extern "C" int zkv_imad_peak(int device, double* wide_per_s, double* fpmul_per_s) {
    if (zkv_device_count() <= device || device < 0) return fail(ZKV_ERR_CUDA, "no such CUDA device");
    CK(cudaSetDevice(device));
    cudaDeviceProp prop; CK(cudaGetDeviceProperties(&prop, device));
    int blocks = prop.multiProcessorCount * 8, threads = 256;
    uint64_t* d_out; fp* d_fp;
    CK(cudaMalloc(&d_out, (size_t)blocks * threads * 8)); CK(cudaMalloc(&d_fp, (size_t)blocks * threads * sizeof(fp)));
    cudaEvent_t e0, e1; CK(cudaEventCreate(&e0)); CK(cudaEventCreate(&e1));
    float best_w = 1e30f, best_f = 1e30f;
    const int it_w = 4096, it_f = 2048;
    for (int rep = 0; rep < 5; rep++) {
        CK(cudaEventRecord(e0)); k_imad_wide<<<blocks, threads>>>((uint32_t*)d_out, 0x9e3779b9u, 0x7f4a7c15u, it_w); CK(cudaEventRecord(e1)); CK(cudaEventSynchronize(e1));
        float ms; CK(cudaEventElapsedTime(&ms, e0, e1)); if (rep) best_w = std::min(best_w, ms);
        CK(cudaEventRecord(e0)); k_fpmul_chain<<<blocks, threads>>>(d_fp, it_f); CK(cudaEventRecord(e1)); CK(cudaEventSynchronize(e1));
        CK(cudaEventElapsedTime(&ms, e0, e1)); if (rep) best_f = std::min(best_f, ms);
    }
    CK(cudaGetLastError());
    if (wide_per_s) *wide_per_s = (double)blocks * threads * it_w * 64.0 / (best_w * 1e-3);
    if (fpmul_per_s) *fpmul_per_s = (double)blocks * threads * it_f * 2.0 / (best_f * 1e-3);
    cudaEventDestroy(e0); cudaEventDestroy(e1); cudaFree(d_out); cudaFree(d_fp);
    return 0;
}
```

Measured before the change: 2.286 million.

## Generate lazy-reduction G2 line functions and prescale f6 in sparse line multiply

Measured after the change: 2.280 million, median of 6. About the same (-0.3%).

```diff
diff --git a/stylus_zkvm_verifiers_b200/csrc/kernels.cuh b/stylus_zkvm_verifiers_b200/csrc/kernels.cuh
--- a/stylus_zkvm_verifiers_b200/csrc/kernels.cuh
+++ b/stylus_zkvm_verifiers_b200/csrc/kernels.cuh
@@ -380,6 +380,24 @@
         case 5: case 6: case 7: lz_frob(A, op - 4); break;
         case 8: { lz_stg12(my + 6, A); for (int s = 0; s < 4; s++) lz_final_exp_stage(s, my + 6, my); break; }
         case 9: lz_st2(L, my[6].c0.c0); lz_st2(L + 2 * LZ_SLOT, my[6].c0.c1); lz_mul_nline(A, X, L); break;
+        case 16: case 17: {
+            const uint32_t RR = tid + LZ_R * LZ_SLOT;
+            for (int k = 0; k < 6; k++) lz_stfp(RR + k * LZ_SLOT, lz_ldfp(A + k * LZ_SLOT));
+            const bool off = !fp_is_zero(my[6].c0.c0.c0);
+            fp* g = &my[0].c0.c0.c0;
+            fp2 a;
+            if (op == 16) { g[0] = lz_ldfp(A + 6 * LZ_SLOT); g[1] = lz_ldfp(A + 7 * LZ_SLOT); a = lz_line_dbl(RR, L, g, g + 1, off); }
+            else { g[0] = lz_ldfp(A + 10 * LZ_SLOT); g[1] = lz_ldfp(A + 11 * LZ_SLOT); a = lz_line_add(RR, L, lz_ld2(A + 6 * LZ_SLOT), lz_ld2(A + 8 * LZ_SLOT), g, g + 1, off); }
+            for (int k = 0; k < 6; k++) lz_stfp(A + k * LZ_SLOT, lz_ldfp(RR + k * LZ_SLOT));
+            lz_st2(A + 6 * LZ_SLOT, a);
+            for (int k = 0; k < 4; k++) lz_stfp(A + (8 + k) * LZ_SLOT, lz_ldfp(L + k * LZ_SLOT));
+            break; }
+        case 18: lz_f6scale(A, lz_ld2(A + 6 * LZ_SLOT)); break;
+        case 19: {
+            nline_t nl; nl.n3 = lz_ld2(A); nl.n4 = lz_ld2(A + 2 * LZ_SLOT);
+            lz_nline_eval(L, nl, lz_ldfp(A + 4 * LZ_SLOT), lz_ldfp(A + 5 * LZ_SLOT));
+            for (int k = 0; k < 4; k++) lz_stfp(A + k * LZ_SLOT, lz_ldfp(L + k * LZ_SLOT));
+            break; }
         default: {
             const fp* yw = &my[6].c0.c0.c0;
             fp* g = &my[0].c0.c0.c0;
diff --git a/stylus_zkvm_verifiers_b200/csrc/lazy.cuh b/stylus_zkvm_verifiers_b200/csrc/lazy.cuh
--- a/stylus_zkvm_verifiers_b200/csrc/lazy.cuh
+++ b/stylus_zkvm_verifiers_b200/csrc/lazy.cuh
@@ -50,8 +50,10 @@
 #endif
 
 LZ_INL void lz_fp_neg(uint32_t* r, const uint32_t* a) { fp z = fp_zero(), x, y; for (int i = 0; i < 8; i++) x.v[i] = a[i]; fp_sub(y, z, x); for (int i = 0; i < 8; i++) r[i] = y.v[i]; }
+LZ_INL void lz_fp_half(uint32_t* r, const uint32_t* a) { fp x, y; for (int i = 0; i < 8; i++) x.v[i] = a[i]; fp_half(y, x); for (int i = 0; i < 8; i++) r[i] = y.v[i]; }
 
 #include "lazy_gen.cuh"
+#include "lazy_g2_gen.cuh"
 
 LZ_INL fp lz_ldfp(uint32_t idx) { fp r; lz_ld(r.v, idx); return r; }
 LZ_INL void lz_stfp(uint32_t idx, const fp& a) { lz_st(idx, a.v); }
@@ -121,7 +123,6 @@
     return r;
 }
 LZ_INL fp2 f2v_neg(const fp2& a) { fp2 r; f2_neg(r, a); return r; }
-LZ_INL fp2 f2v_half(const fp2& a) { fp2 r; f2_half(r, a); return r; }
 LZ_INL fp2 f2v_mul_fp(const fp2& a, const fp& k) { fp2 r; fp_mul(r.c0, a.c0, k); fp_mul(r.c1, a.c1, k); return r; }
 
 LZ_FN2 void lz_mul_line(uint32_t f, uint32_t t, uint32_t l, fp2 a) {
@@ -129,17 +130,18 @@
     { fp6 t1 = lz_f6mul01(f + 6 * LZ_SLOT, l); lz_st6(t, t1); }
     for (int k = 0; k < 3; k++) lz_st2(f + (6 + 2 * k) * LZ_SLOT, f2v_add(lz_ld2(f + 2 * k * LZ_SLOT), lz_ld2(f + (6 + 2 * k) * LZ_SLOT)));
     lz_st2(l, f2v_add(lz_ld2(l), a));
+    lz_f6scale(f, a);
     fp6 s = lz_f6mul01(f + 6 * LZ_SLOT, l);
     {
-        fp2 t0 = f2v_mul(lz_ld2(f), a), t10 = lz_ld2(t), t12 = lz_ld2(t + 4 * LZ_SLOT);
-        lz_st2(f, f2v_add(t0, f2v_xi(t12)));
-        lz_st2(f + 6 * LZ_SLOT, f2v_sub(f2v_sub(s.c0, t0), t10));
-        t0 = f2v_mul(lz_ld2(f + 2 * LZ_SLOT), a); fp2 t11 = lz_ld2(t + 2 * LZ_SLOT);
-        lz_st2(f + 2 * LZ_SLOT, f2v_add(t0, t10));
-        lz_st2(f + 8 * LZ_SLOT, f2v_sub(f2v_sub(s.c1, t0), t11));
-        t0 = f2v_mul(lz_ld2(f + 4 * LZ_SLOT), a);
-        lz_st2(f + 4 * LZ_SLOT, f2v_add(t0, t11));
-        lz_st2(f + 10 * LZ_SLOT, f2v_sub(f2v_sub(s.c2, t0), t12));
+        fp2 t00 = lz_ld2(f), t10 = lz_ld2(t), t12 = lz_ld2(t + 4 * LZ_SLOT);
+        lz_st2(f, f2v_add(t00, f2v_xi(t12)));
+        lz_st2(f + 6 * LZ_SLOT, f2v_sub(f2v_sub(s.c0, t00), t10));
+        fp2 t01 = lz_ld2(f + 2 * LZ_SLOT), t11 = lz_ld2(t + 2 * LZ_SLOT);
+        lz_st2(f + 2 * LZ_SLOT, f2v_add(t01, t10));
+        lz_st2(f + 8 * LZ_SLOT, f2v_sub(f2v_sub(s.c1, t01), t11));
+        fp2 t02 = lz_ld2(f + 4 * LZ_SLOT);
+        lz_st2(f + 4 * LZ_SLOT, f2v_add(t02, t11));
+        lz_st2(f + 10 * LZ_SLOT, f2v_sub(f2v_sub(s.c2, t02), t12));
     }
 }
 
@@ -152,35 +154,6 @@
     }
     lz_st2(l, b); lz_st2(l + 2 * LZ_SLOT, c);
     return a;
-}
-LZ_FN2 fp2 lz_line_dbl(uint32_t r, uint32_t l, const fp* px, const fp* py, bool off) {
-    LZ_RDV();
-    fp2 X = lz_ld2(r), Y = lz_ld2(r + 2 * LZ_SLOT), Z = lz_ld2(r + 4 * LZ_SLOT);
-    fp2 A = f2v_half(f2v_mul(X, Y));
-    fp2 B = f2v_sqr(Y), C = f2v_sqr(Z);
-    fp2 E = f2v_mul(f2_const(C_TWIST_B), f2v_add(f2v_dbl(C), C));
-    fp2 F = f2v_add(f2v_dbl(E), E);
-    fp2 H = f2v_sub(f2v_sqr(f2v_add(Y, Z)), f2v_add(B, C));
-    fp2 J = f2v_sqr(X);
-    fp2 E2 = f2v_sqr(E);
-    lz_st2(r, f2v_mul(A, f2v_sub(B, F)));
-    fp2 G = f2v_sqr(f2v_half(f2v_add(B, F)));
-    lz_st2(r + 2 * LZ_SLOT, f2v_sub(G, f2v_add(f2v_dbl(E2), E2)));
-    lz_st2(r + 4 * LZ_SLOT, f2v_mul(B, H));
-    return lz_line_out(l, f2v_neg(H), f2v_add(f2v_dbl(J), J), f2v_sub(E, B), *px, *py, off);
-}
-LZ_FN2 fp2 lz_line_add(uint32_t r, uint32_t l, fp2 qx, fp2 qy, const fp* px, const fp* py, bool off) {
-    LZ_RDV();
-    fp2 X = lz_ld2(r), Y = lz_ld2(r + 2 * LZ_SLOT), Z = lz_ld2(r + 4 * LZ_SLOT);
-    fp2 th = f2v_sub(Y, f2v_mul(qy, Z)), la = f2v_sub(X, f2v_mul(qx, Z));
-    fp2 C = f2v_sqr(th), D = f2v_sqr(la);
-    fp2 E = f2v_mul(la, D), F = f2v_mul(Z, C), G = f2v_mul(X, D);
-    fp2 H = f2v_sub(f2v_add(E, F), f2v_dbl(G));
-    fp2 l4 = f2v_sub(f2v_mul(th, qx), f2v_mul(la, qy));
-    lz_st2(r + 2 * LZ_SLOT, f2v_sub(f2v_mul(th, f2v_sub(G, H)), f2v_mul(E, Y)));
-    lz_st2(r, f2v_mul(la, H));
-    lz_st2(r + 4 * LZ_SLOT, f2v_mul(Z, E));
-    return lz_line_out(l, la, f2v_neg(th), l4, *px, *py, off);
 }
 
 #define LZ_F 0
@@ -227,8 +200,7 @@
     auto next = lz_line_fetch(in.nt, nx);
     for (int j = 0; j < 2; j++) {
         nline_t nl = lz_line_staged(j);
-        lz_st2(tid + LZ_L * LZ_SLOT, f2v_mul_fp(nl.n3, in.sl[j]));
-        lz_st2(tid + (LZ_L + 2) * LZ_SLOT, f2v_mul_fp(nl.n4, in.sl[2 + j]));
+        lz_nline_eval(tid + LZ_L * LZ_SLOT, nl, in.sl[j], in.sl[2 + j]);
         lz_mul_nline(tid + LZ_F * LZ_SLOT, tid + LZ_T * LZ_SLOT, tid + LZ_L * LZ_SLOT);
     }
     lz_line_stage(next); have = nx == li + 1;
diff --git a/stylus_zkvm_verifiers_b200/csrc/lazy_g2_gen.cuh b/stylus_zkvm_verifiers_b200/csrc/lazy_g2_gen.cuh
--- /dev/null
+++ b/stylus_zkvm_verifiers_b200/csrc/lazy_g2_gen.cuh
@@ -0,0 +1,471 @@
+#pragma once
+
+LZ_FN fp2 lz_line_dbl(uint32_t r, uint32_t l, const fp* px, const fp* py, bool off) {
+    LZ_RDV();
+    uint32_t n1[8]; lz_ld(n1, r + 0 * LZ_SLOT);
+    uint32_t n2[8]; lz_ld(n2, r + 1 * LZ_SLOT);
+    uint32_t n3[8]; lz_ld(n3, r + 2 * LZ_SLOT);
+    uint32_t n4[8]; lz_ld(n4, r + 3 * LZ_SLOT);
+    uint32_t n5[8]; lz_ld(n5, r + 4 * LZ_SLOT);
+    uint32_t n6[8]; lz_ld(n6, r + 5 * LZ_SLOT);
+    uint32_t n7[8]; lz_add8(n7, n3, n4);
+    uint32_t n8[8]; fp_sub_ptx(n8, n3, n4);
+    uint32_t w9[16]; lz_mulw(w9, n7, n8);
+    uint32_t n10[8]; lz_add8(n10, n3, n3);
+    uint32_t w11[16]; lz_mulw(w11, n10, n4);
+    uint32_t n12[8]; lz_add8(n12, n5, n6);
+    uint32_t n13[8]; fp_sub_ptx(n13, n5, n6);
+    uint32_t w14[16]; lz_mulw(w14, n12, n13);
+    uint32_t n15[8]; lz_add8(n15, n5, n5);
+    uint32_t w16[16]; lz_mulw(w16, n15, n6);
+    uint32_t n17[8]; lz_add8(n17, n1, n2);
+    uint32_t n18[8]; fp_sub_ptx(n18, n1, n2);
+    uint32_t w19[16]; lz_mulw(w19, n17, n18);
+    uint32_t n20[8]; lz_add8(n20, n1, n1);
+    uint32_t w21[16]; lz_mulw(w21, n20, n2);
+    uint32_t n22[8]; lz_add8(n22, n1, n2);
+    uint32_t n23[8]; lz_add8(n23, n3, n4);
+    uint32_t w24[16]; lz_mulw(w24, n22, n23);
+    uint32_t w25[16]; lz_mulw(w25, n1, n3);
+    uint32_t w26[16]; lz_subw(w26, w24, w25);
+    uint32_t w27[16]; lz_mulw(w27, n2, n4);
+    uint32_t w28[16]; lz_subw(w28, w26, w27);
+    uint32_t w29[16]; { const uint32_t c_[9] = {0x950d68e5u, 0xeed1e489u, 0x31469cbeu, 0x61fd4f92u, 0xa6fea8bdu, 0xb4dfc389u, 0xaaf2b553u, 0x7c0f83a2u, 0x0925c4b8u}; lz_addhi(w29, w25, c_); }
+    uint32_t w30[16]; lz_subw(w30, w29, w27);
+    uint32_t n31[8]; lz_redc(n31, w9);
+    { const uint32_t k_[8] = {0xd87cfd47u, 0x3c208c16u, 0x6871ca8du, 0x97816a91u, 0x8181585du, 0xb85045b6u, 0xe131a029u, 0x30644e72u}; lz_csub8(n31, n31, k_); }
+    uint32_t n32[8]; lz_redc(n32, w11);
+    { const uint32_t k_[8] = {0xd87cfd47u, 0x3c208c16u, 0x6871ca8du, 0x97816a91u, 0x8181585du, 0xb85045b6u, 0xe131a029u, 0x30644e72u}; lz_csub8(n32, n32, k_); }
+    uint32_t n33[8]; lz_redc(n33, w14);
+    { const uint32_t k_[8] = {0xd87cfd47u, 0x3c208c16u, 0x6871ca8du, 0x97816a91u, 0x8181585du, 0xb85045b6u, 0xe131a029u, 0x30644e72u}; lz_csub8(n33, n33, k_); }
+    uint32_t n34[8]; lz_redc(n34, w16);
+    { const uint32_t k_[8] = {0xd87cfd47u, 0x3c208c16u, 0x6871ca8du, 0x97816a91u, 0x8181585du, 0xb85045b6u, 0xe131a029u, 0x30644e72u}; lz_csub8(n34, n34, k_); }
+    uint32_t w35[16]; lz_addw(w35, w19, w19);
+    uint32_t w36[16]; lz_addw(w36, w35, w19);
+    uint32_t w37[16]; lz_addw(w37, w21, w21);
+    uint32_t w38[16]; lz_addw(w38, w37, w21);
+    uint32_t n39[8]; lz_redc(n39, w36);
+    { const uint32_t k_[8] = {0xb0f9fa8eu, 0x7841182du, 0xd0e3951au, 0x2f02d522u, 0x0302b0bbu, 0x70a08b6du, 0xc2634053u, 0x60c89ce5u}; lz_csub8(n39, n39, k_); }
+    { const uint32_t k_[8] = {0xd87cfd47u, 0x3c208c16u, 0x6871ca8du, 0x97816a91u, 0x8181585du, 0xb85045b6u, 0xe131a029u, 0x30644e72u}; lz_csub8(n39, n39, k_); }
+    uint32_t n40[8]; lz_redc(n40, w38);
+    { const uint32_t k_[8] = {0xb0f9fa8eu, 0x7841182du, 0xd0e3951au, 0x2f02d522u, 0x0302b0bbu, 0x70a08b6du, 0xc2634053u, 0x60c89ce5u}; lz_csub8(n40, n40, k_); }
+    { const uint32_t k_[8] = {0xd87cfd47u, 0x3c208c16u, 0x6871ca8du, 0x97816a91u, 0x8181585du, 0xb85045b6u, 0xe131a029u, 0x30644e72u}; lz_csub8(n40, n40, k_); }
+    uint32_t n41[8]; lz_redc(n41, w30);
+    { const uint32_t k_[8] = {0xd87cfd47u, 0x3c208c16u, 0x6871ca8du, 0x97816a91u, 0x8181585du, 0xb85045b6u, 0xe131a029u, 0x30644e72u}; lz_csub8(n41, n41, k_); }
+    uint32_t n42[8]; lz_redc(n42, w28);
+    { const uint32_t k_[8] = {0xd87cfd47u, 0x3c208c16u, 0x6871ca8du, 0x97816a91u, 0x8181585du, 0xb85045b6u, 0xe131a029u, 0x30644e72u}; lz_csub8(n42, n42, k_); }
+    uint32_t n43[8]; lz_fp_half(n43, n41);
+    uint32_t n44[8]; lz_fp_half(n44, n42);
+    uint32_t n45[8]; fp_add_ptx(n45, n3, n5);
+    uint32_t n46[8]; fp_add_ptx(n46, n4, n6);
+    uint32_t n47[8]; lz_add8(n47, n45, n46);
+    uint32_t n48[8]; fp_sub_ptx(n48, n45, n46);
+    uint32_t w49[16]; lz_mulw(w49, n47, n48);
+    uint32_t n50[8]; lz_add8(n50, n45, n45);
+    uint32_t w51[16]; lz_mulw(w51, n50, n46);
+    const uint32_t k3b0_[8] = {0xb62e0d6au, 0x3baa927cu, 0xd1b664fdu, 0xd71e7c52u, 0xd95d4664u, 0x03873e63u, 0x082ab8f4u, 0x0e75b5b1u};
+    const uint32_t k3b1_[8] = {0x7596fe35u, 0xaab7c666u, 0xbb6a27bau, 0x31d21a78u, 0x680401ffu, 0x85dd7297u, 0xdf39a7e9u, 0x03c52d6au};
+    uint32_t n52[8]; lz_add8(n52, k3b0_, k3b1_);
+    uint32_t n53[8]; lz_add8(n53, n33, n34);
+    uint32_t w54[16]; lz_mulw(w54, n52, n53);
+    uint32_t w55[16]; lz_mulw(w55, k3b0_, n33);
+    uint32_t w56[16]; lz_subw(w56, w54, w55);
+    uint32_t w57[16]; lz_mulw(w57, k3b1_, n34);
+    uint32_t w58[16]; lz_subw(w58, w56, w57);
+    uint32_t w59[16]; { const uint32_t c_[9] = {0x950d68e5u, 0xeed1e489u, 0x31469cbeu, 0x61fd4f92u, 0xa6fea8bdu, 0xb4dfc389u, 0xaaf2b553u, 0x7c0f83a2u, 0x0925c4b8u}; lz_addhi(w59, w55, c_); }
+    uint32_t w60[16]; lz_subw(w60, w59, w57);
+    uint32_t n61[8]; lz_redc(n61, w60);
+    { const uint32_t k_[8] = {0xd87cfd47u, 0x3c208c16u, 0x6871ca8du, 0x97816a91u, 0x8181585du, 0xb85045b6u, 0xe131a029u, 0x30644e72u}; lz_csub8(n61, n61, k_); }
+    uint32_t n62[8]; lz_redc(n62, w58);
+    { const uint32_t k_[8] = {0xd87cfd47u, 0x3c208c16u, 0x6871ca8du, 0x97816a91u, 0x8181585du, 0xb85045b6u, 0xe131a029u, 0x30644e72u}; lz_csub8(n62, n62, k_); }
+    uint32_t w63[16]; { const uint32_t c_[9] = {0x2a1ad1cau, 0xdda3c913u, 0x628d397du, 0xc3fa9f24u, 0x4dfd517au, 0x69bf8713u, 0x55e56aa7u, 0xf81f0745u, 0x124b8970u}; lz_addhi(w63, w49, c_); }
+    uint32_t w64[16]; lz_subw(w64, w63, w9);
+    uint32_t w65[16]; { const uint32_t c_[9] = {0x2a1ad1cau, 0xdda3c913u, 0x628d397du, 0xc3fa9f24u, 0x4dfd517au, 0x69bf8713u, 0x55e56aa7u, 0xf81f0745u, 0x124b8970u}; lz_addhi(w65, w51, c_); }
+    uint32_t w66[16]; lz_subw(w66, w65, w11);
+    uint32_t w67[16]; { const uint32_t c_[9] = {0x2a1ad1cau, 0xdda3c913u, 0x628d397du, 0xc3fa9f24u, 0x4dfd517au, 0x69bf8713u, 0x55e56aa7u, 0xf81f0745u, 0x124b8970u}; lz_addhi(w67, w64, c_); }
+    uint32_t w68[16]; lz_subw(w68, w67, w14);
+    uint32_t w69[16]; { const uint32_t c_[9] = {0x2a1ad1cau, 0xdda3c913u, 0x628d397du, 0xc3fa9f24u, 0x4dfd517au, 0x69bf8713u, 0x55e56aa7u, 0xf81f0745u, 0x124b8970u}; lz_addhi(w69, w66, c_); }
+    uint32_t w70[16]; lz_subw(w70, w69, w16);
+    uint32_t n71[8]; lz_redc(n71, w68);
+    { const uint32_t k_[8] = {0xb0f9fa8eu, 0x7841182du, 0xd0e3951au, 0x2f02d522u, 0x0302b0bbu, 0x70a08b6du, 0xc2634053u, 0x60c89ce5u}; lz_csub8(n71, n71, k_); }
+    { const uint32_t k_[8] = {0xd87cfd47u, 0x3c208c16u, 0x6871ca8du, 0x97816a91u, 0x8181585du, 0xb85045b6u, 0xe131a029u, 0x30644e72u}; lz_csub8(n71, n71, k_); }
+    uint32_t n72[8]; lz_redc(n72, w70);
+    { const uint32_t k_[8] = {0xb0f9fa8eu, 0x7841182du, 0xd0e3951au, 0x2f02d522u, 0x0302b0bbu, 0x70a08b6du, 0xc2634053u, 0x60c89ce5u}; lz_csub8(n72, n72, k_); }
+    { const uint32_t k_[8] = {0xd87cfd47u, 0x3c208c16u, 0x6871ca8du, 0x97816a91u, 0x8181585du, 0xb85045b6u, 0xe131a029u, 0x30644e72u}; lz_csub8(n72, n72, k_); }
+    uint32_t n73[8]; fp_add_ptx(n73, n61, n61);
+    uint32_t n74[8]; fp_add_ptx(n74, n62, n62);
+    uint32_t n75[8]; fp_add_ptx(n75, n73, n61);
+    uint32_t n76[8]; fp_add_ptx(n76, n74, n62);
+    uint32_t n77[8]; fp_add_ptx(n77, n31, n75);
+    uint32_t n78[8]; fp_add_ptx(n78, n32, n76);
+    uint32_t n79[8]; lz_fp_half(n79, n77);
+    uint32_t n80[8]; lz_fp_half(n80, n78);
+    uint32_t n81[8]; lz_add8(n81, n61, n62);
+    uint32_t n82[8]; fp_sub_ptx(n82, n61, n62);
+    uint32_t w83[16]; lz_mulw(w83, n81, n82);
+    uint32_t n84[8]; lz_add8(n84, n61, n61);
+    uint32_t w85[16]; lz_mulw(w85, n84, n62);
+    uint32_t n86[8]; lz_add8(n86, n79, n80);
+    uint32_t n87[8]; fp_sub_ptx(n87, n79, n80);
+    uint32_t w88[16]; lz_mulw(w88, n86, n87);
+    uint32_t n89[8]; lz_add8(n89, n79, n79);
+    uint32_t w90[16]; lz_mulw(w90, n89, n80);
+    uint32_t w91[16]; lz_addw(w91, w83, w83);
+    uint32_t w92[16]; lz_addw(w92, w91, w83);
+    uint32_t w93[16]; lz_addw(w93, w85, w85);
+    uint32_t w94[16]; lz_addw(w94, w93, w85);
+    uint32_t w95[16]; { const uint32_t c_[9] = {0x7e50755eu, 0x98eb5b39u, 0x27a7ac79u, 0x4befdd6du, 0xe9f7f470u, 0x3d3e9539u, 0x01b03ff6u, 0xe85d15d0u, 0x36e29c52u}; lz_addhi(w95, w88, c_); }
+    uint32_t w96[16]; lz_subw(w96, w95, w92);
+    uint32_t w97[16]; { const uint32_t c_[9] = {0x7e50755eu, 0x98eb5b39u, 0x27a7ac79u, 0x4befdd6du, 0xe9f7f470u, 0x3d3e9539u, 0x01b03ff6u, 0xe85d15d0u, 0x36e29c52u}; lz_addhi(w97, w90, c_); }
+    uint32_t w98[16]; lz_subw(w98, w97, w94);
+    uint32_t n99[8]; lz_redc(n99, w96);
+    { const uint32_t k_[8] = {0xb0f9fa8eu, 0x7841182du, 0xd0e3951au, 0x2f02d522u, 0x0302b0bbu, 0x70a08b6du, 0xc2634053u, 0x60c89ce5u}; lz_csub8(n99, n99, k_); }
+    { const uint32_t k_[8] = {0xd87cfd47u, 0x3c208c16u, 0x6871ca8du, 0x97816a91u, 0x8181585du, 0xb85045b6u, 0xe131a029u, 0x30644e72u}; lz_csub8(n99, n99, k_); }
+    uint32_t n100[8]; lz_redc(n100, w98);
+    { const uint32_t k_[8] = {0xb0f9fa8eu, 0x7841182du, 0xd0e3951au, 0x2f02d522u, 0x0302b0bbu, 0x70a08b6du, 0xc2634053u, 0x60c89ce5u}; lz_csub8(n100, n100, k_); }
+    { const uint32_t k_[8] = {0xd87cfd47u, 0x3c208c16u, 0x6871ca8du, 0x97816a91u, 0x8181585du, 0xb85045b6u, 0xe131a029u, 0x30644e72u}; lz_csub8(n100, n100, k_); }
+    uint32_t n101[8]; fp_sub_ptx(n101, n31, n75);
+    uint32_t n102[8]; fp_sub_ptx(n102, n32, n76);
+    uint32_t n103[8]; lz_add8(n103, n43, n44);
+    uint32_t n104[8]; lz_add8(n104, n101, n102);
+    uint32_t w105[16]; lz_mulw(w105, n103, n104);
+    uint32_t w106[16]; lz_mulw(w106, n43, n101);
+    uint32_t w107[16]; lz_subw(w107, w105, w106);
+    uint32_t w108[16]; lz_mulw(w108, n44, n102);
+    uint32_t w109[16]; lz_subw(w109, w107, w108);
+    uint32_t w110[16]; { const uint32_t c_[9] = {0x950d68e5u, 0xeed1e489u, 0x31469cbeu, 0x61fd4f92u, 0xa6fea8bdu, 0xb4dfc389u, 0xaaf2b553u, 0x7c0f83a2u, 0x0925c4b8u}; lz_addhi(w110, w106, c_); }
+    uint32_t w111[16]; lz_subw(w111, w110, w108);
+    uint32_t n112[8]; lz_redc(n112, w111);
+    { const uint32_t k_[8] = {0xd87cfd47u, 0x3c208c16u, 0x6871ca8du, 0x97816a91u, 0x8181585du, 0xb85045b6u, 0xe131a029u, 0x30644e72u}; lz_csub8(n112, n112, k_); }
+    uint32_t n113[8]; lz_redc(n113, w109);
+    { const uint32_t k_[8] = {0xd87cfd47u, 0x3c208c16u, 0x6871ca8du, 0x97816a91u, 0x8181585du, 0xb85045b6u, 0xe131a029u, 0x30644e72u}; lz_csub8(n113, n113, k_); }
+    uint32_t n114[8]; lz_add8(n114, n31, n32);
+    uint32_t n115[8]; lz_add8(n115, n71, n72);
+    uint32_t w116[16]; lz_mulw(w116, n114, n115);
+    uint32_t w117[16]; lz_mulw(w117, n31, n71);
+    uint32_t w118[16]; lz_subw(w118, w116, w117);
+    uint32_t w119[16]; lz_mulw(w119, n32, n72);
+    uint32_t w120[16]; lz_subw(w120, w118, w119);
+    uint32_t w121[16]; { const uint32_t c_[9] = {0x950d68e5u, 0xeed1e489u, 0x31469cbeu, 0x61fd4f92u, 0xa6fea8bdu, 0xb4dfc389u, 0xaaf2b553u, 0x7c0f83a2u, 0x0925c4b8u}; lz_addhi(w121, w117, c_); }
+    uint32_t w122[16]; lz_subw(w122, w121, w119);
+    uint32_t n123[8]; lz_redc(n123, w122);
+    { const uint32_t k_[8] = {0xd87cfd47u, 0x3c208c16u, 0x6871ca8du, 0x97816a91u, 0x8181585du, 0xb85045b6u, 0xe131a029u, 0x30644e72u}; lz_csub8(n123, n123, k_); }
+    uint32_t n124[8]; lz_redc(n124, w120);
+    { const uint32_t k_[8] = {0xd87cfd47u, 0x3c208c16u, 0x6871ca8du, 0x97816a91u, 0x8181585du, 0xb85045b6u, 0xe131a029u, 0x30644e72u}; lz_csub8(n124, n124, k_); }
+    uint32_t n125[8]; lz_fp_neg(n125, n71);
+    uint32_t n126[8]; lz_fp_neg(n126, n72);
+    uint32_t w127[16]; lz_mulw(w127, n125, py->v);
+    uint32_t n128[8]; lz_redc(n128, w127);
+    { const uint32_t k_[8] = {0xd87cfd47u, 0x3c208c16u, 0x6871ca8du, 0x97816a91u, 0x8181585du, 0xb85045b6u, 0xe131a029u, 0x30644e72u}; lz_csub8(n128, n128, k_); }
+    uint32_t w129[16]; lz_mulw(w129, n126, py->v);
+    uint32_t n130[8]; lz_redc(n130, w129);
+    { const uint32_t k_[8] = {0xd87cfd47u, 0x3c208c16u, 0x6871ca8du, 0x97816a91u, 0x8181585du, 0xb85045b6u, 0xe131a029u, 0x30644e72u}; lz_csub8(n130, n130, k_); }
+    uint32_t w131[16]; lz_mulw(w131, n39, px->v);
+    uint32_t n132[8]; lz_redc(n132, w131);
+    { const uint32_t k_[8] = {0xd87cfd47u, 0x3c208c16u, 0x6871ca8du, 0x97816a91u, 0x8181585du, 0xb85045b6u, 0xe131a029u, 0x30644e72u}; lz_csub8(n132, n132, k_); }
+    uint32_t w133[16]; lz_mulw(w133, n40, px->v);
+    uint32_t n134[8]; lz_redc(n134, w133);
+    { const uint32_t k_[8] = {0xd87cfd47u, 0x3c208c16u, 0x6871ca8du, 0x97816a91u, 0x8181585du, 0xb85045b6u, 0xe131a029u, 0x30644e72u}; lz_csub8(n134, n134, k_); }
+    uint32_t n135[8]; fp_sub_ptx(n135, n61, n31);
+    uint32_t n136[8]; fp_sub_ptx(n136, n62, n32);
+    lz_st(r + 0 * LZ_SLOT, n112);
+    lz_st(r + 1 * LZ_SLOT, n113);
+    lz_st(r + 2 * LZ_SLOT, n99);
+    lz_st(r + 3 * LZ_SLOT, n100);
+    lz_st(r + 4 * LZ_SLOT, n123);
+    lz_st(r + 5 * LZ_SLOT, n124);
+    const uint32_t keep_ = off ? 0u : 0xffffffffu;
+    fp2 r_;
+    for (int i_ = 0; i_ < 8; i_++) {
+        r_.c0.v[i_] = (n128[i_] & keep_) | (C_ONE[i_] & ~keep_); r_.c1.v[i_] = n130[i_] & keep_;
+        n132[i_] &= keep_; n134[i_] &= keep_; n135[i_] &= keep_; n136[i_] &= keep_;
+    }
+    lz_st(l, n132); lz_st(l + LZ_SLOT, n134); lz_st(l + 2 * LZ_SLOT, n135); lz_st(l + 3 * LZ_SLOT, n136);
+    return r_;
+}
+
+LZ_FN fp2 lz_line_add(uint32_t r, uint32_t l, fp2 qx, fp2 qy, const fp* px, const fp* py, bool off) {
+    LZ_RDV();
+    uint32_t n1[8]; lz_ld(n1, r + 0 * LZ_SLOT);
+    uint32_t n2[8]; lz_ld(n2, r + 1 * LZ_SLOT);
+    uint32_t n3[8]; lz_ld(n3, r + 2 * LZ_SLOT);
+    uint32_t n4[8]; lz_ld(n4, r + 3 * LZ_SLOT);
+    uint32_t n5[8]; lz_ld(n5, r + 4 * LZ_SLOT);
+    uint32_t n6[8]; lz_ld(n6, r + 5 * LZ_SLOT);
+    uint32_t n7[8]; lz_add8(n7, qy.c0.v, qy.c1.v);
+    uint32_t n8[8]; lz_add8(n8, n5, n6);
+    uint32_t w9[16]; lz_mulw(w9, n7, n8);
+    uint32_t w10[16]; lz_mulw(w10, qy.c0.v, n5);
+    uint32_t w11[16]; lz_subw(w11, w9, w10);
+    uint32_t w12[16]; lz_mulw(w12, qy.c1.v, n6);
+    uint32_t w13[16]; lz_subw(w13, w11, w12);
+    uint32_t w14[16]; { const uint32_t c_[9] = {0x950d68e5u, 0xeed1e489u, 0x31469cbeu, 0x61fd4f92u, 0xa6fea8bdu, 0xb4dfc389u, 0xaaf2b553u, 0x7c0f83a2u, 0x0925c4b8u}; lz_addhi(w14, w10, c_); }
+    uint32_t w15[16]; lz_subw(w15, w14, w12);
+    uint32_t n16[8]; lz_redc(n16, w15);
+    { const uint32_t k_[8] = {0xd87cfd47u, 0x3c208c16u, 0x6871ca8du, 0x97816a91u, 0x8181585du, 0xb85045b6u, 0xe131a029u, 0x30644e72u}; lz_csub8(n16, n16, k_); }
+    uint32_t n17[8]; lz_redc(n17, w13);
+    { const uint32_t k_[8] = {0xd87cfd47u, 0x3c208c16u, 0x6871ca8du, 0x97816a91u, 0x8181585du, 0xb85045b6u, 0xe131a029u, 0x30644e72u}; lz_csub8(n17, n17, k_); }
+    uint32_t n18[8]; lz_add8(n18, qx.c0.v, qx.c1.v);
+    uint32_t n19[8]; lz_add8(n19, n5, n6);
+    uint32_t w20[16]; lz_mulw(w20, n18, n19);
+    uint32_t w21[16]; lz_mulw(w21, qx.c0.v, n5);
+    uint32_t w22[16]; lz_subw(w22, w20, w21);
+    uint32_t w23[16]; lz_mulw(w23, qx.c1.v, n6);
+    uint32_t w24[16]; lz_subw(w24, w22, w23);
+    uint32_t w25[16]; { const uint32_t c_[9] = {0x950d68e5u, 0xeed1e489u, 0x31469cbeu, 0x61fd4f92u, 0xa6fea8bdu, 0xb4dfc389u, 0xaaf2b553u, 0x7c0f83a2u, 0x0925c4b8u}; lz_addhi(w25, w21, c_); }
+    uint32_t w26[16]; lz_subw(w26, w25, w23);
+    uint32_t n27[8]; lz_redc(n27, w26);
+    { const uint32_t k_[8] = {0xd87cfd47u, 0x3c208c16u, 0x6871ca8du, 0x97816a91u, 0x8181585du, 0xb85045b6u, 0xe131a029u, 0x30644e72u}; lz_csub8(n27, n27, k_); }
+    uint32_t n28[8]; lz_redc(n28, w24);
+    { const uint32_t k_[8] = {0xd87cfd47u, 0x3c208c16u, 0x6871ca8du, 0x97816a91u, 0x8181585du, 0xb85045b6u, 0xe131a029u, 0x30644e72u}; lz_csub8(n28, n28, k_); }
+    uint32_t n29[8]; fp_sub_ptx(n29, n3, n16);
+    uint32_t n30[8]; fp_sub_ptx(n30, n4, n17);
+    uint32_t n31[8]; fp_sub_ptx(n31, n1, n27);
+    uint32_t n32[8]; fp_sub_ptx(n32, n2, n28);
+    uint32_t n33[8]; lz_add8(n33, n29, n30);
+    uint32_t n34[8]; fp_sub_ptx(n34, n29, n30);
+    uint32_t w35[16]; lz_mulw(w35, n33, n34);
+    uint32_t n36[8]; lz_add8(n36, n29, n29);
+    uint32_t w37[16]; lz_mulw(w37, n36, n30);
+    uint32_t n38[8]; lz_add8(n38, n31, n32);
+    uint32_t n39[8]; fp_sub_ptx(n39, n31, n32);
+    uint32_t w40[16]; lz_mulw(w40, n38, n39);
+    uint32_t n41[8]; lz_add8(n41, n31, n31);
+    uint32_t w42[16]; lz_mulw(w42, n41, n32);
+    uint32_t n43[8]; lz_redc(n43, w35);
+    { const uint32_t k_[8] = {0xd87cfd47u, 0x3c208c16u, 0x6871ca8du, 0x97816a91u, 0x8181585du, 0xb85045b6u, 0xe131a029u, 0x30644e72u}; lz_csub8(n43, n43, k_); }
+    uint32_t n44[8]; lz_redc(n44, w37);
+    { const uint32_t k_[8] = {0xd87cfd47u, 0x3c208c16u, 0x6871ca8du, 0x97816a91u, 0x8181585du, 0xb85045b6u, 0xe131a029u, 0x30644e72u}; lz_csub8(n44, n44, k_); }
+    uint32_t n45[8]; lz_redc(n45, w40);
+    { const uint32_t k_[8] = {0xd87cfd47u, 0x3c208c16u, 0x6871ca8du, 0x97816a91u, 0x8181585du, 0xb85045b6u, 0xe131a029u, 0x30644e72u}; lz_csub8(n45, n45, k_); }
+    uint32_t n46[8]; lz_redc(n46, w42);
+    { const uint32_t k_[8] = {0xd87cfd47u, 0x3c208c16u, 0x6871ca8du, 0x97816a91u, 0x8181585du, 0xb85045b6u, 0xe131a029u, 0x30644e72u}; lz_csub8(n46, n46, k_); }
+    uint32_t n47[8]; lz_add8(n47, n31, n32);
+    uint32_t n48[8]; lz_add8(n48, n45, n46);
+    uint32_t w49[16]; lz_mulw(w49, n47, n48);
+    uint32_t w50[16]; lz_mulw(w50, n31, n45);
+    uint32_t w51[16]; lz_subw(w51, w49, w50);
+    uint32_t w52[16]; lz_mulw(w52, n32, n46);
+    uint32_t w53[16]; lz_subw(w53, w51, w52);
+    uint32_t w54[16]; { const uint32_t c_[9] = {0x950d68e5u, 0xeed1e489u, 0x31469cbeu, 0x61fd4f92u, 0xa6fea8bdu, 0xb4dfc389u, 0xaaf2b553u, 0x7c0f83a2u, 0x0925c4b8u}; lz_addhi(w54, w50, c_); }
+    uint32_t w55[16]; lz_subw(w55, w54, w52);
+    uint32_t n56[8]; lz_add8(n56, n1, n2);
+    uint32_t n57[8]; lz_add8(n57, n45, n46);
+    uint32_t w58[16]; lz_mulw(w58, n56, n57);
+    uint32_t w59[16]; lz_mulw(w59, n1, n45);
+    uint32_t w60[16]; lz_subw(w60, w58, w59);
+    uint32_t w61[16]; lz_mulw(w61, n2, n46);
+    uint32_t w62[16]; lz_subw(w62, w60, w61);
+    uint32_t w63[16]; { const uint32_t c_[9] = {0x950d68e5u, 0xeed1e489u, 0x31469cbeu, 0x61fd4f92u, 0xa6fea8bdu, 0xb4dfc389u, 0xaaf2b553u, 0x7c0f83a2u, 0x0925c4b8u}; lz_addhi(w63, w59, c_); }
+    uint32_t w64[16]; lz_subw(w64, w63, w61);
+    uint32_t n65[8]; lz_add8(n65, n5, n6);
+    uint32_t n66[8]; lz_add8(n66, n43, n44);
+    uint32_t w67[16]; lz_mulw(w67, n65, n66);
+    uint32_t w68[16]; lz_mulw(w68, n5, n43);
+    uint32_t w69[16]; lz_subw(w69, w67, w68);
+    uint32_t w70[16]; lz_mulw(w70, n6, n44);
+    uint32_t w71[16]; lz_subw(w71, w69, w70);
+    uint32_t w72[16]; { const uint32_t c_[9] = {0x950d68e5u, 0xeed1e489u, 0x31469cbeu, 0x61fd4f92u, 0xa6fea8bdu, 0xb4dfc389u, 0xaaf2b553u, 0x7c0f83a2u, 0x0925c4b8u}; lz_addhi(w72, w68, c_); }
+    uint32_t w73[16]; lz_subw(w73, w72, w70);
+    uint32_t n74[8]; lz_add8(n74, n29, n30);
+    uint32_t n75[8]; lz_add8(n75, qx.c0.v, qx.c1.v);
+    uint32_t w76[16]; lz_mulw(w76, n74, n75);
+    uint32_t w77[16]; lz_mulw(w77, n29, qx.c0.v);
+    uint32_t w78[16]; lz_subw(w78, w76, w77);
+    uint32_t w79[16]; lz_mulw(w79, n30, qx.c1.v);
+    uint32_t w80[16]; lz_subw(w80, w78, w79);
+    uint32_t w81[16]; { const uint32_t c_[9] = {0x950d68e5u, 0xeed1e489u, 0x31469cbeu, 0x61fd4f92u, 0xa6fea8bdu, 0xb4dfc389u, 0xaaf2b553u, 0x7c0f83a2u, 0x0925c4b8u}; lz_addhi(w81, w77, c_); }
+    uint32_t w82[16]; lz_subw(w82, w81, w79);
+    uint32_t n83[8]; lz_add8(n83, n31, n32);
+    uint32_t n84[8]; lz_add8(n84, qy.c0.v, qy.c1.v);
+    uint32_t w85[16]; lz_mulw(w85, n83, n84);
+    uint32_t w86[16]; lz_mulw(w86, n31, qy.c0.v);
+    uint32_t w87[16]; lz_subw(w87, w85, w86);
+    uint32_t w88[16]; lz_mulw(w88, n32, qy.c1.v);
+    uint32_t w89[16]; lz_subw(w89, w87, w88);
+    uint32_t w90[16]; { const uint32_t c_[9] = {0x950d68e5u, 0xeed1e489u, 0x31469cbeu, 0x61fd4f92u, 0xa6fea8bdu, 0xb4dfc389u, 0xaaf2b553u, 0x7c0f83a2u, 0x0925c4b8u}; lz_addhi(w90, w86, c_); }
+    uint32_t w91[16]; lz_subw(w91, w90, w88);
+    uint32_t w92[16]; { const uint32_t c_[9] = {0x2a1ad1cau, 0xdda3c913u, 0x628d397du, 0xc3fa9f24u, 0x4dfd517au, 0x69bf8713u, 0x55e56aa7u, 0xf81f0745u, 0x124b8970u}; lz_addhi(w92, w82, c_); }
+    uint32_t w93[16]; lz_subw(w93, w92, w91);
+    uint32_t w94[16]; { const uint32_t c_[9] = {0x2a1ad1cau, 0xdda3c913u, 0x628d397du, 0xc3fa9f24u, 0x4dfd517au, 0x69bf8713u, 0x55e56aa7u, 0xf81f0745u, 0x124b8970u}; lz_addhi(w94, w80, c_); }
+    uint32_t w95[16]; lz_subw(w95, w94, w89);
+    uint32_t n96[8]; lz_redc(n96, w55);
+    { const uint32_t k_[8] = {0xd87cfd47u, 0x3c208c16u, 0x6871ca8du, 0x97816a91u, 0x8181585du, 0xb85045b6u, 0xe131a029u, 0x30644e72u}; lz_csub8(n96, n96, k_); }
+    uint32_t n97[8]; lz_redc(n97, w53);
+    { const uint32_t k_[8] = {0xd87cfd47u, 0x3c208c16u, 0x6871ca8du, 0x97816a91u, 0x8181585du, 0xb85045b6u, 0xe131a029u, 0x30644e72u}; lz_csub8(n97, n97, k_); }
+    uint32_t n98[8]; lz_redc(n98, w64);
+    { const uint32_t k_[8] = {0xd87cfd47u, 0x3c208c16u, 0x6871ca8du, 0x97816a91u, 0x8181585du, 0xb85045b6u, 0xe131a029u, 0x30644e72u}; lz_csub8(n98, n98, k_); }
+    uint32_t n99[8]; lz_redc(n99, w62);
+    { const uint32_t k_[8] = {0xd87cfd47u, 0x3c208c16u, 0x6871ca8du, 0x97816a91u, 0x8181585du, 0xb85045b6u, 0xe131a029u, 0x30644e72u}; lz_csub8(n99, n99, k_); }
+    uint32_t w100[16]; lz_addw(w100, w55, w73);
+    uint32_t w101[16]; lz_addw(w101, w53, w71);
+    uint32_t w102[16]; lz_addw(w102, w64, w64);
+    uint32_t w103[16]; lz_addw(w103, w62, w62);
+    uint32_t w104[16]; { const uint32_t c_[9] = {0x5435a394u, 0xbb479226u, 0xc51a72fbu, 0x87f53e48u, 0x9bfaa2f5u, 0xd37f0e26u, 0xabcad54eu, 0xf03e0e8au, 0x249712e1u}; lz_addhi(w104, w100, c_); }
+    uint32_t w105[16]; lz_subw(w105, w104, w102);
+    uint32_t w106[16]; { const uint32_t c_[9] = {0x5435a394u, 0xbb479226u, 0xc51a72fbu, 0x87f53e48u, 0x9bfaa2f5u, 0xd37f0e26u, 0xabcad54eu, 0xf03e0e8au, 0x249712e1u}; lz_addhi(w106, w101, c_); }
+    uint32_t w107[16]; lz_subw(w107, w106, w103);
+    uint32_t n108[8]; lz_redc(n108, w105);
+    { const uint32_t k_[8] = {0xb0f9fa8eu, 0x7841182du, 0xd0e3951au, 0x2f02d522u, 0x0302b0bbu, 0x70a08b6du, 0xc2634053u, 0x60c89ce5u}; lz_csub8(n108, n108, k_); }
+    { const uint32_t k_[8] = {0xd87cfd47u, 0x3c208c16u, 0x6871ca8du, 0x97816a91u, 0x8181585du, 0xb85045b6u, 0xe131a029u, 0x30644e72u}; lz_csub8(n108, n108, k_); }
+    uint32_t n109[8]; lz_redc(n109, w107);
+    { const uint32_t k_[8] = {0xb0f9fa8eu, 0x7841182du, 0xd0e3951au, 0x2f02d522u, 0x0302b0bbu, 0x70a08b6du, 0xc2634053u, 0x60c89ce5u}; lz_csub8(n109, n109, k_); }
+    { const uint32_t k_[8] = {0xd87cfd47u, 0x3c208c16u, 0x6871ca8du, 0x97816a91u, 0x8181585du, 0xb85045b6u, 0xe131a029u, 0x30644e72u}; lz_csub8(n109, n109, k_); }
+    uint32_t n110[8]; lz_redc(n110, w93);
+    { const uint32_t k_[8] = {0xd87cfd47u, 0x3c208c16u, 0x6871ca8du, 0x97816a91u, 0x8181585du, 0xb85045b6u, 0xe131a029u, 0x30644e72u}; lz_csub8(n110, n110, k_); }
+    uint32_t n111[8]; lz_redc(n111, w95);
+    { const uint32_t k_[8] = {0xd87cfd47u, 0x3c208c16u, 0x6871ca8du, 0x97816a91u, 0x8181585du, 0xb85045b6u, 0xe131a029u, 0x30644e72u}; lz_csub8(n111, n111, k_); }
+    uint32_t n112[8]; fp_sub_ptx(n112, n98, n108);
+    uint32_t n113[8]; fp_sub_ptx(n113, n99, n109);
+    uint32_t n114[8]; lz_add8(n114, n29, n30);
+    uint32_t n115[8]; lz_add8(n115, n112, n113);
+    uint32_t w116[16]; lz_mulw(w116, n114, n115);
+    uint32_t w117[16]; lz_mulw(w117, n29, n112);
+    uint32_t w118[16]; lz_subw(w118, w116, w117);
+    uint32_t w119[16]; lz_mulw(w119, n30, n113);
+    uint32_t w120[16]; lz_subw(w120, w118, w119);
+    uint32_t w121[16]; { const uint32_t c_[9] = {0x950d68e5u, 0xeed1e489u, 0x31469cbeu, 0x61fd4f92u, 0xa6fea8bdu, 0xb4dfc389u, 0xaaf2b553u, 0x7c0f83a2u, 0x0925c4b8u}; lz_addhi(w121, w117, c_); }
+    uint32_t w122[16]; lz_subw(w122, w121, w119);
+    uint32_t n123[8]; lz_add8(n123, n96, n97);
+    uint32_t n124[8]; lz_add8(n124, n3, n4);
+    uint32_t w125[16]; lz_mulw(w125, n123, n124);
+    uint32_t w126[16]; lz_mulw(w126, n96, n3);
+    uint32_t w127[16]; lz_subw(w127, w125, w126);
+    uint32_t w128[16]; lz_mulw(w128, n97, n4);
+    uint32_t w129[16]; lz_subw(w129, w127, w128);
+    uint32_t w130[16]; { const uint32_t c_[9] = {0x950d68e5u, 0xeed1e489u, 0x31469cbeu, 0x61fd4f92u, 0xa6fea8bdu, 0xb4dfc389u, 0xaaf2b553u, 0x7c0f83a2u, 0x0925c4b8u}; lz_addhi(w130, w126, c_); }
+    uint32_t w131[16]; lz_subw(w131, w130, w128);
+    uint32_t w132[16]; { const uint32_t c_[9] = {0x2a1ad1cau, 0xdda3c913u, 0x628d397du, 0xc3fa9f24u, 0x4dfd517au, 0x69bf8713u, 0x55e56aa7u, 0xf81f0745u, 0x124b8970u}; lz_addhi(w132, w122, c_); }
+    uint32_t w133[16]; lz_subw(w133, w132, w131);
+    uint32_t w134[16]; { const uint32_t c_[9] = {0x2a1ad1cau, 0xdda3c913u, 0x628d397du, 0xc3fa9f24u, 0x4dfd517au, 0x69bf8713u, 0x55e56aa7u, 0xf81f0745u, 0x124b8970u}; lz_addhi(w134, w120, c_); }
+    uint32_t w135[16]; lz_subw(w135, w134, w129);
+    uint32_t n136[8]; lz_redc(n136, w133);
+    { const uint32_t k_[8] = {0xd87cfd47u, 0x3c208c16u, 0x6871ca8du, 0x97816a91u, 0x8181585du, 0xb85045b6u, 0xe131a029u, 0x30644e72u}; lz_csub8(n136, n136, k_); }
+    uint32_t n137[8]; lz_redc(n137, w135);
+    { const uint32_t k_[8] = {0xd87cfd47u, 0x3c208c16u, 0x6871ca8du, 0x97816a91u, 0x8181585du, 0xb85045b6u, 0xe131a029u, 0x30644e72u}; lz_csub8(n137, n137, k_); }
+    uint32_t n138[8]; lz_add8(n138, n31, n32);
+    uint32_t n139[8]; lz_add8(n139, n108, n109);
+    uint32_t w140[16]; lz_mulw(w140, n138, n139);
+    uint32_t w141[16]; lz_mulw(w141, n31, n108);
+    uint32_t w142[16]; lz_subw(w142, w140, w141);
+    uint32_t w143[16]; lz_mulw(w143, n32, n109);
+    uint32_t w144[16]; lz_subw(w144, w142, w143);
+    uint32_t w145[16]; { const uint32_t c_[9] = {0x950d68e5u, 0xeed1e489u, 0x31469cbeu, 0x61fd4f92u, 0xa6fea8bdu, 0xb4dfc389u, 0xaaf2b553u, 0x7c0f83a2u, 0x0925c4b8u}; lz_addhi(w145, w141, c_); }
+    uint32_t w146[16]; lz_subw(w146, w145, w143);
+    uint32_t n147[8]; lz_redc(n147, w146);
+    { const uint32_t k_[8] = {0xd87cfd47u, 0x3c208c16u, 0x6871ca8du, 0x97816a91u, 0x8181585du, 0xb85045b6u, 0xe131a029u, 0x30644e72u}; lz_csub8(n147, n147, k_); }
+    uint32_t n148[8]; lz_redc(n148, w144);
+    { const uint32_t k_[8] = {0xd87cfd47u, 0x3c208c16u, 0x6871ca8du, 0x97816a91u, 0x8181585du, 0xb85045b6u, 0xe131a029u, 0x30644e72u}; lz_csub8(n148, n148, k_); }
+    uint32_t n149[8]; lz_add8(n149, n5, n6);
+    uint32_t n150[8]; lz_add8(n150, n96, n97);
+    uint32_t w151[16]; lz_mulw(w151, n149, n150);
+    uint32_t w152[16]; lz_mulw(w152, n5, n96);
+    uint32_t w153[16]; lz_subw(w153, w151, w152);
+    uint32_t w154[16]; lz_mulw(w154, n6, n97);
+    uint32_t w155[16]; lz_subw(w155, w153, w154);
+    uint32_t w156[16]; { const uint32_t c_[9] = {0x950d68e5u, 0xeed1e489u, 0x31469cbeu, 0x61fd4f92u, 0xa6fea8bdu, 0xb4dfc389u, 0xaaf2b553u, 0x7c0f83a2u, 0x0925c4b8u}; lz_addhi(w156, w152, c_); }
+    uint32_t w157[16]; lz_subw(w157, w156, w154);
+    uint32_t n158[8]; lz_redc(n158, w157);
+    { const uint32_t k_[8] = {0xd87cfd47u, 0x3c208c16u, 0x6871ca8du, 0x97816a91u, 0x8181585du, 0xb85045b6u, 0xe131a029u, 0x30644e72u}; lz_csub8(n158, n158, k_); }
+    uint32_t n159[8]; lz_redc(n159, w155);
+    { const uint32_t k_[8] = {0xd87cfd47u, 0x3c208c16u, 0x6871ca8du, 0x97816a91u, 0x8181585du, 0xb85045b6u, 0xe131a029u, 0x30644e72u}; lz_csub8(n159, n159, k_); }
+    uint32_t n160[8]; lz_fp_neg(n160, n29);
+    uint32_t n161[8]; lz_fp_neg(n161, n30);
+    uint32_t w162[16]; lz_mulw(w162, n31, py->v);
+    uint32_t n163[8]; lz_redc(n163, w162);
+    { const uint32_t k_[8] = {0xd87cfd47u, 0x3c208c16u, 0x6871ca8du, 0x97816a91u, 0x8181585du, 0xb85045b6u, 0xe131a029u, 0x30644e72u}; lz_csub8(n163, n163, k_); }
+    uint32_t w164[16]; lz_mulw(w164, n32, py->v);
+    uint32_t n165[8]; lz_redc(n165, w164);
+    { const uint32_t k_[8] = {0xd87cfd47u, 0x3c208c16u, 0x6871ca8du, 0x97816a91u, 0x8181585du, 0xb85045b6u, 0xe131a029u, 0x30644e72u}; lz_csub8(n165, n165, k_); }
+    uint32_t w166[16]; lz_mulw(w166, n160, px->v);
+    uint32_t n167[8]; lz_redc(n167, w166);
+    { const uint32_t k_[8] = {0xd87cfd47u, 0x3c208c16u, 0x6871ca8du, 0x97816a91u, 0x8181585du, 0xb85045b6u, 0xe131a029u, 0x30644e72u}; lz_csub8(n167, n167, k_); }
+    uint32_t w168[16]; lz_mulw(w168, n161, px->v);
+    uint32_t n169[8]; lz_redc(n169, w168);
+    { const uint32_t k_[8] = {0xd87cfd47u, 0x3c208c16u, 0x6871ca8du, 0x97816a91u, 0x8181585du, 0xb85045b6u, 0xe131a029u, 0x30644e72u}; lz_csub8(n169, n169, k_); }
+    lz_st(r + 0 * LZ_SLOT, n147);
+    lz_st(r + 1 * LZ_SLOT, n148);
+    lz_st(r + 2 * LZ_SLOT, n136);
+    lz_st(r + 3 * LZ_SLOT, n137);
+    lz_st(r + 4 * LZ_SLOT, n158);
+    lz_st(r + 5 * LZ_SLOT, n159);
+    const uint32_t keep_ = off ? 0u : 0xffffffffu;
+    fp2 r_;
+    for (int i_ = 0; i_ < 8; i_++) {
+        r_.c0.v[i_] = (n163[i_] & keep_) | (C_ONE[i_] & ~keep_); r_.c1.v[i_] = n165[i_] & keep_;
+        n167[i_] &= keep_; n169[i_] &= keep_; n110[i_] &= keep_; n111[i_] &= keep_;
+    }
+    lz_st(l, n167); lz_st(l + LZ_SLOT, n169); lz_st(l + 2 * LZ_SLOT, n110); lz_st(l + 3 * LZ_SLOT, n111);
+    return r_;
+}
+
+LZ_FN void lz_f6scale(uint32_t f, fp2 a) {
+    uint32_t n1[8]; lz_ld(n1, f + 0 * LZ_SLOT);
+    uint32_t n2[8]; lz_ld(n2, f + 1 * LZ_SLOT);
+    uint32_t n3[8]; lz_ld(n3, f + 2 * LZ_SLOT);
+    uint32_t n4[8]; lz_ld(n4, f + 3 * LZ_SLOT);
+    uint32_t n5[8]; lz_ld(n5, f + 4 * LZ_SLOT);
+    uint32_t n6[8]; lz_ld(n6, f + 5 * LZ_SLOT);
+    uint32_t n7[8]; lz_add8(n7, a.c0.v, a.c1.v);
+    uint32_t n8[8]; lz_add8(n8, n1, n2);
+    uint32_t w9[16]; lz_mulw(w9, n8, n7);
+    uint32_t w10[16]; lz_mulw(w10, n1, a.c0.v);
+    uint32_t w11[16]; lz_mulw(w11, n2, a.c1.v);
+    uint32_t w12[16]; { const uint32_t c_[9] = {0x950d68e5u, 0xeed1e489u, 0x31469cbeu, 0x61fd4f92u, 0xa6fea8bdu, 0xb4dfc389u, 0xaaf2b553u, 0x7c0f83a2u, 0x0925c4b8u}; lz_addhi(w12, w10, c_); }
+    uint32_t w13[16]; lz_subw(w13, w12, w11);
+    uint32_t w14[16]; lz_subw(w14, w9, w10);
+    uint32_t w15[16]; lz_subw(w15, w14, w11);
+    uint32_t n16[8]; lz_redc(n16, w13);
+    { const uint32_t k_[8] = {0xd87cfd47u, 0x3c208c16u, 0x6871ca8du, 0x97816a91u, 0x8181585du, 0xb85045b6u, 0xe131a029u, 0x30644e72u}; lz_csub8(n16, n16, k_); }
+    uint32_t n17[8]; lz_redc(n17, w15);
+    { const uint32_t k_[8] = {0xd87cfd47u, 0x3c208c16u, 0x6871ca8du, 0x97816a91u, 0x8181585du, 0xb85045b6u, 0xe131a029u, 0x30644e72u}; lz_csub8(n17, n17, k_); }
+    uint32_t n18[8]; lz_add8(n18, n3, n4);
+    uint32_t w19[16]; lz_mulw(w19, n18, n7);
+    uint32_t w20[16]; lz_mulw(w20, n3, a.c0.v);
+    uint32_t w21[16]; lz_mulw(w21, n4, a.c1.v);
+    uint32_t w22[16]; { const uint32_t c_[9] = {0x950d68e5u, 0xeed1e489u, 0x31469cbeu, 0x61fd4f92u, 0xa6fea8bdu, 0xb4dfc389u, 0xaaf2b553u, 0x7c0f83a2u, 0x0925c4b8u}; lz_addhi(w22, w20, c_); }
+    uint32_t w23[16]; lz_subw(w23, w22, w21);
+    uint32_t w24[16]; lz_subw(w24, w19, w20);
+    uint32_t w25[16]; lz_subw(w25, w24, w21);
+    uint32_t n26[8]; lz_redc(n26, w23);
+    { const uint32_t k_[8] = {0xd87cfd47u, 0x3c208c16u, 0x6871ca8du, 0x97816a91u, 0x8181585du, 0xb85045b6u, 0xe131a029u, 0x30644e72u}; lz_csub8(n26, n26, k_); }
+    uint32_t n27[8]; lz_redc(n27, w25);
+    { const uint32_t k_[8] = {0xd87cfd47u, 0x3c208c16u, 0x6871ca8du, 0x97816a91u, 0x8181585du, 0xb85045b6u, 0xe131a029u, 0x30644e72u}; lz_csub8(n27, n27, k_); }
+    uint32_t n28[8]; lz_add8(n28, n5, n6);
+    uint32_t w29[16]; lz_mulw(w29, n28, n7);
+    uint32_t w30[16]; lz_mulw(w30, n5, a.c0.v);
+    uint32_t w31[16]; lz_mulw(w31, n6, a.c1.v);
+    uint32_t w32[16]; { const uint32_t c_[9] = {0x950d68e5u, 0xeed1e489u, 0x31469cbeu, 0x61fd4f92u, 0xa6fea8bdu, 0xb4dfc389u, 0xaaf2b553u, 0x7c0f83a2u, 0x0925c4b8u}; lz_addhi(w32, w30, c_); }
+    uint32_t w33[16]; lz_subw(w33, w32, w31);
+    uint32_t w34[16]; lz_subw(w34, w29, w30);
+    uint32_t w35[16]; lz_subw(w35, w34, w31);
+    uint32_t n36[8]; lz_redc(n36, w33);
+    { const uint32_t k_[8] = {0xd87cfd47u, 0x3c208c16u, 0x6871ca8du, 0x97816a91u, 0x8181585du, 0xb85045b6u, 0xe131a029u, 0x30644e72u}; lz_csub8(n36, n36, k_); }
+    uint32_t n37[8]; lz_redc(n37, w35);
+    { const uint32_t k_[8] = {0xd87cfd47u, 0x3c208c16u, 0x6871ca8du, 0x97816a91u, 0x8181585du, 0xb85045b6u, 0xe131a029u, 0x30644e72u}; lz_csub8(n37, n37, k_); }
+    lz_st(f + 0 * LZ_SLOT, n16);
+    lz_st(f + 1 * LZ_SLOT, n17);
+    lz_st(f + 2 * LZ_SLOT, n26);
+    lz_st(f + 3 * LZ_SLOT, n27);
+    lz_st(f + 4 * LZ_SLOT, n36);
+    lz_st(f + 5 * LZ_SLOT, n37);
+}
+
+LZ_FN void lz_nline_eval(uint32_t l, nline_t nl, fp s, fp t) {
+    uint32_t w1[16]; lz_mulw(w1, nl.n3.c0.v, s.v);
+    uint32_t n2[8]; lz_redc(n2, w1);
+    { const uint32_t k_[8] = {0xd87cfd47u, 0x3c208c16u, 0x6871ca8du, 0x97816a91u, 0x8181585du, 0xb85045b6u, 0xe131a029u, 0x30644e72u}; lz_csub8(n2, n2, k_); }
+    uint32_t w3[16]; lz_mulw(w3, nl.n3.c1.v, s.v);
+    uint32_t n4[8]; lz_redc(n4, w3);
+    { const uint32_t k_[8] = {0xd87cfd47u, 0x3c208c16u, 0x6871ca8du, 0x97816a91u, 0x8181585du, 0xb85045b6u, 0xe131a029u, 0x30644e72u}; lz_csub8(n4, n4, k_); }
+    uint32_t w5[16]; lz_mulw(w5, nl.n4.c0.v, t.v);
+    uint32_t n6[8]; lz_redc(n6, w5);
+    { const uint32_t k_[8] = {0xd87cfd47u, 0x3c208c16u, 0x6871ca8du, 0x97816a91u, 0x8181585du, 0xb85045b6u, 0xe131a029u, 0x30644e72u}; lz_csub8(n6, n6, k_); }
+    uint32_t w7[16]; lz_mulw(w7, nl.n4.c1.v, t.v);
+    uint32_t n8[8]; lz_redc(n8, w7);
+    { const uint32_t k_[8] = {0xd87cfd47u, 0x3c208c16u, 0x6871ca8du, 0x97816a91u, 0x8181585du, 0xb85045b6u, 0xe131a029u, 0x30644e72u}; lz_csub8(n8, n8, k_); }
+    lz_st(l + 0 * LZ_SLOT, n2);
+    lz_st(l + 1 * LZ_SLOT, n4);
+    lz_st(l + 2 * LZ_SLOT, n6);
+    lz_st(l + 3 * LZ_SLOT, n8);
+}
diff --git a/stylus_zkvm_verifiers_b200/csrc/zkv.cu b/stylus_zkvm_verifiers_b200/csrc/zkv.cu
--- a/stylus_zkvm_verifiers_b200/csrc/zkv.cu
+++ b/stylus_zkvm_verifiers_b200/csrc/zkv.cu
@@ -1024,7 +1024,8 @@
 extern "C" int zkv_fp12_op_batch(int op, const uint8_t* a, const uint8_t* b, size_t n, uint8_t* out, int device) {
     const bool slots = op >= 16;
     const int k = slots ? op - 16 : op;
-    if (!a || !out || k < 0 || k > (slots ? 10 : 9) || ((k == 0 || k == 2 || k == 9 || k == 10) && !b)) return fail(ZKV_ERR_ARG, "zkv_fp12_op_batch: bad argument");
+    if (!a || !out || k < 0 || (k > (slots ? 10 : 9) && !(slots && k >= 16 && k <= 19)) || ((k == 0 || k == 2 || k == 9 || k == 10) && !b))
+        return fail(ZKV_ERR_ARG, "zkv_fp12_op_batch: bad argument");
     if (n == 0) return 0;
     uint8_t dummy;
     if (!slots)
```
